# gabrieletiboni/random-envs

Hardware: NVIDIA B200
Metric: DR env-steps/sec (RandomCartPole-v0 single-step kernel, uniform DR resample on reset) (higher is better)
Workload: dtype f32

## Files before the change

### include/renv.h

```cpp
#ifndef RENV_B200_H
#define RENV_B200_H

#include <stdint.h>

#ifdef __cplusplus
extern "C" {
#endif

#define RENV_ABI_VERSION 6
#define RENV_MAX_DIM 32
#define RENV_NUM_STATS 6
#define RENV_TILE_ENVS_F32 1024
#define RENV_TILE_ENVS_F64 512
#define RENV_NUM_COUNTERS 3

enum renv_status {
    RENV_OK = 0,
    RENV_E_NULL = -1,
    RENV_E_ALIGN = -2,
    RENV_E_SIZE = -3,
    RENV_E_DIM = -4,
    RENV_E_DRTYPE = -5,
    RENV_E_INTEGRATOR = -6,
    RENV_E_ARG = -7
};

enum renv_dr_type {
    RENV_DR_NONE = 0,
    RENV_DR_UNIFORM = 1,
    RENV_DR_TRUNCNORM = 2,
    RENV_DR_GAUSSIAN = 3,
    RENV_DR_FULLGAUSSIAN = 4
};

enum renv_integrator { RENV_EULER = 0, RENV_SEMI_IMPLICIT = 1 };

typedef struct renv_dr_cfg {
    int32_t dr_type;
    int32_t dim;
    double a[RENV_MAX_DIM];
    double b[RENV_MAX_DIM];
    double lb[RENV_MAX_DIM];
    double factor[RENV_MAX_DIM * RENV_MAX_DIM];
} renv_dr_cfg;

typedef struct renv_cartpole_env {
    void *state;
    void *xi;
    int32_t *elapsed;
    uint32_t *episode;
    int32_t *beyond;
    uint16_t *elapsed16;
    uint32_t *progress;
    int64_t n;
    int64_t ld;
    uint64_t env_id0;
    uint64_t seed;
} renv_cartpole_env;

typedef struct renv_episode_log {
    void *xi;
    void *final_state;
    int32_t *length;
    uint8_t *truncated;
    int64_t *end_tick;
    int32_t *count;
    int64_t capacity;
} renv_episode_log;

int renv_abi_version(void);
const char *renv_strerror(int code);

int renv_dr_sample_f32(float *out, int64_t n, const renv_dr_cfg *cfg, uint64_t seed, uint64_t sample_id0,
                       uint32_t call, unsigned long long *violations, void *stream);
int renv_dr_sample_f64(double *out, int64_t n, const renv_dr_cfg *cfg, uint64_t seed, uint64_t sample_id0,
                       uint32_t call, unsigned long long *violations, void *stream);

int renv_cartpole_reset_f32(const renv_cartpole_env *env, const uint8_t *mask, uint64_t tick, const renv_dr_cfg *dr,
                            unsigned long long *violations, void *stream);
int renv_cartpole_reset_f64(const renv_cartpole_env *env, const uint8_t *mask, uint64_t tick, const renv_dr_cfg *dr,
                            unsigned long long *violations, void *stream);

int renv_cartpole_step_f32(const renv_cartpole_env *env, const uint8_t *action, float *reward, uint8_t *done,
                           uint8_t *truncated, int integrator, int max_steps, int auto_reset, uint64_t tick,
                           const renv_dr_cfg *dr, unsigned long long *counters, void *stream);
int renv_cartpole_step_f64(const renv_cartpole_env *env, const uint8_t *action, double *reward, uint8_t *done,
                           uint8_t *truncated, int integrator, int max_steps, int auto_reset, uint64_t tick,
                           const renv_dr_cfg *dr, unsigned long long *counters, void *stream);

int renv_cartpole_step_lean_f32(const renv_cartpole_env *env, const uint8_t *action, uint8_t *done, uint8_t *truncated,
                                int integrator, int max_steps, uint64_t tick, const renv_dr_cfg *dr,
                                unsigned long long *counters, void *stream);

typedef struct renv_obs_noise {
    void *obs;
    double std;
} renv_obs_noise;

int renv_cartpole_reset_noisy_f32(const renv_cartpole_env *env, const renv_obs_noise *noise, const uint8_t *mask,
                                  uint64_t tick, const renv_dr_cfg *dr, unsigned long long *violations, void *stream);
int renv_cartpole_reset_noisy_f64(const renv_cartpole_env *env, const renv_obs_noise *noise, const uint8_t *mask,
                                  uint64_t tick, const renv_dr_cfg *dr, unsigned long long *violations, void *stream);
int renv_cartpole_step_noisy_f32(const renv_cartpole_env *env, const renv_obs_noise *noise, const uint8_t *action,
                                 float *reward, uint8_t *done, uint8_t *truncated, int integrator, int max_steps,
                                 int auto_reset, uint64_t tick, const renv_dr_cfg *dr, unsigned long long *counters,
                                 void *stream);
int renv_cartpole_step_noisy_f64(const renv_cartpole_env *env, const renv_obs_noise *noise, const uint8_t *action,
                                 double *reward, uint8_t *done, uint8_t *truncated, int integrator, int max_steps,
                                 int auto_reset, uint64_t tick, const renv_dr_cfg *dr, unsigned long long *counters,
                                 void *stream);

int renv_cartpole_rollout_f32(const renv_cartpole_env *env, const double w[4], double b, int K, int integrator,
                              int max_steps, uint64_t tick, const renv_dr_cfg *dr, double *stats,
                              unsigned long long *violations, void *stream);
int renv_cartpole_rollout_f64(const renv_cartpole_env *env, const double w[4], double b, int K, int integrator,
                              int max_steps, uint64_t tick, const renv_dr_cfg *dr, double *stats,
                              unsigned long long *violations, void *stream);

int renv_cartpole_rollout_noisy_f32(const renv_cartpole_env *env, const renv_obs_noise *noise, const double w[4], double b,
                                    int K, int integrator, int max_steps, uint64_t tick, const renv_dr_cfg *dr,
                                    double *stats, unsigned long long *violations, void *stream);
int renv_cartpole_rollout_noisy_f64(const renv_cartpole_env *env, const renv_obs_noise *noise, const double w[4], double b,
                                    int K, int integrator, int max_steps, uint64_t tick, const renv_dr_cfg *dr,
                                    double *stats, unsigned long long *violations, void *stream);

int renv_cartpole_step_logged_f32(const renv_cartpole_env *env, const renv_episode_log *log, const uint8_t *action,
                                  float *reward, uint8_t *done, uint8_t *truncated, int integrator, int max_steps,
                                  uint64_t tick, const renv_dr_cfg *dr, unsigned long long *counters, void *stream);
int renv_cartpole_step_logged_f64(const renv_cartpole_env *env, const renv_episode_log *log, const uint8_t *action,
                                  double *reward, uint8_t *done, uint8_t *truncated, int integrator, int max_steps,
                                  uint64_t tick, const renv_dr_cfg *dr, unsigned long long *counters, void *stream);
int renv_cartpole_rollout_logged_f32(const renv_cartpole_env *env, const renv_episode_log *log, const double w[4], double b,
                                     int K, int integrator, int max_steps, uint64_t tick, const renv_dr_cfg *dr,
                                     double *stats, unsigned long long *violations, void *stream);
int renv_cartpole_rollout_logged_f64(const renv_cartpole_env *env, const renv_episode_log *log, const double w[4], double b,
                                     int K, int integrator, int max_steps, uint64_t tick, const renv_dr_cfg *dr,
                                     double *stats, unsigned long long *violations, void *stream);

#define RENV_MLP_HIDDEN 64
#define RENV_MLP_PARAM_FLOATS 4612
#define RENV_MLP_TANH 0
#define RENV_MLP_RELU 1
typedef struct renv_mlp_policy {
    const void *params;
    int32_t activation;
} renv_mlp_policy;

int renv_cartpole_policy_actions_mlp_f32(const renv_cartpole_env *env, const renv_mlp_policy *p, uint8_t *action,
                                         float *logits, void *stream);
int renv_cartpole_rollout_mlp_f32(const renv_cartpole_env *env, const renv_mlp_policy *p, int K, int integrator,
                                  int max_steps, uint64_t tick, const renv_dr_cfg *dr, double *stats,
                                  unsigned long long *violations, void *stream);
int renv_cartpole_rollout_mlp_logged_f32(const renv_cartpole_env *env, const renv_episode_log *log,
                                         const renv_mlp_policy *p, int K, int integrator, int max_steps, uint64_t tick,
                                         const renv_dr_cfg *dr, double *stats, unsigned long long *violations,
                                         void *stream);

int renv_cartpole_policy_logp_mlp_f32(const renv_cartpole_env *env, const renv_mlp_policy *p, int sample, uint64_t tick,
                                      uint8_t *action, float *logp, float *logits, void *stream);

typedef struct renv_trajectory {
    float *obs;
    uint8_t *action;
    uint8_t *done;
    float *logp;
    uint8_t *truncated;
    float *final_obs;
    int32_t capacity;
} renv_trajectory;

int renv_cartpole_collect_mlp_f32(const renv_cartpole_env *env, const renv_mlp_policy *p, const renv_trajectory *traj,
                                  int sample, int K, int integrator, int max_steps, uint64_t tick, const renv_dr_cfg *dr,
                                  double *stats, unsigned long long *violations, void *stream);
int renv_cartpole_collect_mlp_logged_f32(const renv_cartpole_env *env, const renv_episode_log *log,
                                         const renv_mlp_policy *p, const renv_trajectory *traj, int sample, int K,
                                         int integrator, int max_steps, uint64_t tick, const renv_dr_cfg *dr,
                                         double *stats, unsigned long long *violations, void *stream);

#define RENV_SCALAR_SAVE_BYTES 512
typedef struct renv_scalar_ctrl {
    uint32_t request;
    uint32_t pad0[15];
    double arg[16];
    uint64_t arg_u64[8];
    double state[4];
    double obs[4];
    double xi[4];
    double reward;
    int32_t done;
    int32_t beyond;
    uint32_t violations;
    uint32_t pad1;
    uint32_t ack;
    uint32_t exited;
    uint32_t pad2[16];
    struct renv_scalar_outcome {
        double state[4];
        double obs[4];
        double reward;
        int32_t done;
        int32_t beyond;
        uint32_t pad[12];
    } next[2];
    uint32_t next_seq;
    uint32_t pad3[15];
} renv_scalar_ctrl;
int renv_cartpole_scalar_serve(renv_scalar_ctrl *ctrl, void *save, uint32_t lease_id, uint64_t lease_ns, void *stream);

int renv_random_actions_u8(uint8_t *action, int64_t n, uint64_t env_id0, uint64_t seed, uint32_t step,
                           void *stream);

int renv_pack_flags_u8(const uint8_t *flags, uint32_t *bits, int64_t n, void *stream);

#ifdef __cplusplus
}
#endif
#endif
```

### random_envs_b200/_lib.py

```python
import ctypes
import os

_HERE = os.path.dirname(os.path.abspath(__file__))
LIB_PATH = os.environ.get("RENV_B200_LIB", os.path.join(_HERE, "librenv_b200.so"))

ABI_VERSION = 6
MAX_DIM = 32
NUM_STATS = 6
SCALAR_SAVE_BYTES = 512
COUNTER_GAUSSIAN, COUNTER_BAD_ACTION, COUNTER_ORDER_TIMEOUT = 0, 1, 2
TILE_ENVS = {'float32': 1024, 'float64': 512}
NUM_COUNTERS = 3

OK = 0
DR_NONE, DR_UNIFORM, DR_TRUNCNORM, DR_GAUSSIAN, DR_FULLGAUSSIAN = 0, 1, 2, 3, 4
DR_TYPE_IDS = {"uniform": DR_UNIFORM, "truncnorm": DR_TRUNCNORM, "gaussian": DR_GAUSSIAN,
               "fullgaussian": DR_FULLGAUSSIAN}
EULER, SEMI_IMPLICIT = 0, 1


class DrCfg(ctypes.Structure):
    _fields_ = [("dr_type", ctypes.c_int32), ("dim", ctypes.c_int32),
                ("a", ctypes.c_double * MAX_DIM), ("b", ctypes.c_double * MAX_DIM),
                ("lb", ctypes.c_double * MAX_DIM), ("factor", ctypes.c_double * (MAX_DIM * MAX_DIM))]


class CartpoleEnv(ctypes.Structure):
    _fields_ = [("state", ctypes.c_void_p), ("xi", ctypes.c_void_p), ("elapsed", ctypes.c_void_p),
                ("episode", ctypes.c_void_p), ("beyond", ctypes.c_void_p), ("elapsed16", ctypes.c_void_p),
                ("progress", ctypes.c_void_p),
                ("n", ctypes.c_int64), ("ld", ctypes.c_int64),
                ("env_id0", ctypes.c_uint64), ("seed", ctypes.c_uint64)]


class ObsNoise(ctypes.Structure):
    _fields_ = [("obs", ctypes.c_void_p), ("std", ctypes.c_double)]


class EpisodeLog(ctypes.Structure):
    _fields_ = [("xi", ctypes.c_void_p), ("final_state", ctypes.c_void_p), ("length", ctypes.c_void_p),
                ("truncated", ctypes.c_void_p), ("end_tick", ctypes.c_void_p), ("count", ctypes.c_void_p),
                ("capacity", ctypes.c_int64)]


class MlpPolicy(ctypes.Structure):
    _fields_ = [("params", ctypes.c_void_p), ("activation", ctypes.c_int32)]


class Trajectory(ctypes.Structure):
    _fields_ = [("obs", ctypes.c_void_p), ("action", ctypes.c_void_p), ("done", ctypes.c_void_p),
                ("logp", ctypes.c_void_p), ("truncated", ctypes.c_void_p), ("final_obs", ctypes.c_void_p),
                ("capacity", ctypes.c_int32)]


_vp, _i64, _u64, _u32, _int, _dbl = (ctypes.c_void_p, ctypes.c_int64, ctypes.c_uint64, ctypes.c_uint32,
                                     ctypes.c_int, ctypes.c_double)
_cfg_p, _env_p, _noise_p = ctypes.POINTER(DrCfg), ctypes.POINTER(CartpoleEnv), ctypes.POINTER(ObsNoise)
_log_p = ctypes.POINTER(EpisodeLog)
_mlp_p = ctypes.POINTER(MlpPolicy)
_traj_p = ctypes.POINTER(Trajectory)

SIGNATURES = {
    "renv_abi_version": (_int, []),
    "renv_strerror": (ctypes.c_char_p, [_int]),
    "renv_dr_sample_f32": (_int, [_vp, _i64, _cfg_p, _u64, _u64, _u32, _vp, _vp]),
    "renv_dr_sample_f64": (_int, [_vp, _i64, _cfg_p, _u64, _u64, _u32, _vp, _vp]),
    "renv_cartpole_reset_f32": (_int, [_env_p, _vp, _u64, _cfg_p, _vp, _vp]),
    "renv_cartpole_reset_f64": (_int, [_env_p, _vp, _u64, _cfg_p, _vp, _vp]),
    "renv_cartpole_step_f32": (_int, [_env_p, _vp, _vp, _vp, _vp, _int, _int, _int, _u64, _cfg_p, _vp, _vp]),
    "renv_cartpole_step_f64": (_int, [_env_p, _vp, _vp, _vp, _vp, _int, _int, _int, _u64, _cfg_p, _vp, _vp]),
    "renv_cartpole_step_lean_f32": (_int, [_env_p, _vp, _vp, _vp, _int, _int, _u64, _cfg_p, _vp, _vp]),
    "renv_cartpole_reset_noisy_f32": (_int, [_env_p, _noise_p, _vp, _u64, _cfg_p, _vp, _vp]),
    "renv_cartpole_reset_noisy_f64": (_int, [_env_p, _noise_p, _vp, _u64, _cfg_p, _vp, _vp]),
    "renv_cartpole_step_noisy_f32": (_int, [_env_p, _noise_p, _vp, _vp, _vp, _vp, _int, _int, _int, _u64, _cfg_p, _vp, _vp]),
    "renv_cartpole_step_noisy_f64": (_int, [_env_p, _noise_p, _vp, _vp, _vp, _vp, _int, _int, _int, _u64, _cfg_p, _vp, _vp]),
    "renv_cartpole_rollout_f32": (_int, [_env_p, ctypes.POINTER(_dbl), _dbl, _int, _int, _int, _u64, _cfg_p, _vp, _vp, _vp]),
    "renv_cartpole_rollout_f64": (_int, [_env_p, ctypes.POINTER(_dbl), _dbl, _int, _int, _int, _u64, _cfg_p, _vp, _vp, _vp]),
    "renv_cartpole_rollout_noisy_f32": (_int, [_env_p, _noise_p, ctypes.POINTER(_dbl), _dbl, _int, _int, _int, _u64, _cfg_p, _vp, _vp, _vp]),
    "renv_cartpole_rollout_noisy_f64": (_int, [_env_p, _noise_p, ctypes.POINTER(_dbl), _dbl, _int, _int, _int, _u64, _cfg_p, _vp, _vp, _vp]),
    "renv_cartpole_step_logged_f32": (_int, [_env_p, _log_p, _vp, _vp, _vp, _vp, _int, _int, _u64, _cfg_p, _vp, _vp]),
    "renv_cartpole_step_logged_f64": (_int, [_env_p, _log_p, _vp, _vp, _vp, _vp, _int, _int, _u64, _cfg_p, _vp, _vp]),
    "renv_cartpole_rollout_logged_f32": (_int, [_env_p, _log_p, ctypes.POINTER(_dbl), _dbl, _int, _int, _int, _u64, _cfg_p, _vp, _vp, _vp]),
    "renv_cartpole_rollout_logged_f64": (_int, [_env_p, _log_p, ctypes.POINTER(_dbl), _dbl, _int, _int, _int, _u64, _cfg_p, _vp, _vp, _vp]),
    "renv_cartpole_policy_actions_mlp_f32": (_int, [_env_p, _mlp_p, _vp, _vp, _vp]),
    "renv_cartpole_rollout_mlp_f32": (_int, [_env_p, _mlp_p, _int, _int, _int, _u64, _cfg_p, _vp, _vp, _vp]),
    "renv_cartpole_rollout_mlp_logged_f32": (_int, [_env_p, _log_p, _mlp_p, _int, _int, _int, _u64, _cfg_p, _vp, _vp, _vp]),
    "renv_cartpole_policy_logp_mlp_f32": (_int, [_env_p, _mlp_p, _int, _u64, _vp, _vp, _vp, _vp]),
    "renv_cartpole_collect_mlp_f32": (_int, [_env_p, _mlp_p, _traj_p, _int, _int, _int, _int, _u64, _cfg_p, _vp, _vp, _vp]),
    "renv_cartpole_collect_mlp_logged_f32": (_int, [_env_p, _log_p, _mlp_p, _traj_p, _int, _int, _int, _int, _u64, _cfg_p,
                                                    _vp, _vp, _vp]),
    "renv_cartpole_scalar_serve": (_int, [_vp, _vp, _u32, _u64, _vp]),
    "renv_random_actions_u8": (_int, [_vp, _i64, _u64, _u64, _u32, _vp]),
    "renv_pack_flags_u8": (_int, [_vp, _vp, _i64, _vp]),
}


class RenvError(RuntimeError):

    def __init__(self, fn, code, message):
        super().__init__("%s failed with %d: %s" % (fn, code, message))
        self.code = code


_lib = None


def load():
    global _lib
    if _lib is not None:
        return _lib
    if not os.path.isfile(LIB_PATH):
        raise ImportError(
            "random_envs_b200: %s is missing. Build it with `python -m random_envs_b200.build` "
            "(needs nvcc; sm_100a). There is no CPU fallback." % LIB_PATH)
    lib = ctypes.CDLL(LIB_PATH)
    for name, (restype, argtypes) in SIGNATURES.items():
        try:
            fn = getattr(lib, name)
        except AttributeError as exc:
            raise ImportError("random_envs_b200: symbol %s missing from %s" % (name, LIB_PATH)) from exc
        fn.restype, fn.argtypes = restype, argtypes
    if lib.renv_abi_version() != ABI_VERSION:
        raise ImportError("random_envs_b200: ABI version mismatch (library %d, binding %d); rebuild"
                          % (lib.renv_abi_version(), ABI_VERSION))
    _lib = lib
    return lib


def strerror(code):
    return load().renv_strerror(code).decode()


def call(name, *args):
    rc = getattr(load(), name)(*args)
    if rc != OK:
        raise RenvError(name, rc, strerror(rc))


def make_dr_cfg(dr_type, a, b, lb=None, factor=None):
    cfg = DrCfg()
    if dr_type is None:
        cfg.dr_type, cfg.dim = DR_NONE, 0
        return cfg
    if dr_type not in DR_TYPE_IDS:
        raise Exception("Unknown dr_type:" + str(dr_type))
    dim = len(a)
    if not 1 <= dim <= MAX_DIM:
        raise ValueError("task_dim %d outside [1, %d]" % (dim, MAX_DIM))
    cfg.dr_type, cfg.dim = DR_TYPE_IDS[dr_type], dim
    for i in range(dim):
        cfg.a[i] = float(a[i])
        cfg.b[i] = float(b[i])
        cfg.lb[i] = float(lb[i]) if lb is not None else 0.0
    if factor is not None:
        for i in range(dim):
            for k in range(dim):
                cfg.factor[i * dim + k] = float(factor[i][k])
    return cfg
```

### random_envs_b200/csrc/renv_abi.cu

```cuda
#include "../../include/renv.h"
#include "renv_kernels.cuh"
#include <cmath>
#include "renv_rollout_pair.cuh"
#include "renv_fullgauss_tc.cuh"
#include "renv_mlp_policy.cuh"
#include "renv_scalar_server.cuh"
#include <stdlib.h>

#ifndef RENV_ROLLOUT_F32_PAIR
#define RENV_ROLLOUT_F32_PAIR 1
#endif

using namespace renv;

namespace {

inline bool aligned(const void *p, size_t a) { return (reinterpret_cast<uintptr_t>(p) & (a - 1)) == 0; }

template <typename T> int to_cfg4(const renv_dr_cfg *dr, DrCfg4<T> *out)
{
    out->dr_type = kDrNone;
    out->dim = 4;
    for (int k = 0; k < 4; ++k) { out->a[k] = T(0); out->b[k] = T(0); out->floor[k] = T(0); }
    for (int k = 0; k < 16; ++k) out->factor[k] = T(0);
    if (dr == nullptr || dr->dr_type == RENV_DR_NONE) return RENV_OK;
    if (dr->dr_type < RENV_DR_NONE || dr->dr_type > RENV_DR_FULLGAUSSIAN) return RENV_E_DRTYPE;
    if (dr->dim != 4) return RENV_E_DIM;
    out->dr_type = dr->dr_type;
    for (int k = 0; k < 4; ++k) {
        const T a = (T)dr->a[k], b = (T)dr->b[k];
        out->a[k] = a;
        if (dr->dr_type == RENV_DR_UNIFORM) {
            const T width = b - a;
            out->b[k] = sizeof(T) == 4 ? (T)(width * (T)(1.0 / 16777216.0)) : width;
            out->floor[k] = T(0);
        } else if (dr->dr_type == RENV_DR_FULLGAUSSIAN) {
            out->b[k] = b;
            out->floor[k] = (T)dr->lb[k];
        } else {
            out->b[k] = b;
            out->floor[k] = dr->dr_type == RENV_DR_TRUNCNORM ? (T)dr->lb[k] : (T)0.1;
        }
    }
    if (dr->dr_type == RENV_DR_FULLGAUSSIAN)
        for (int k = 0; k < 16; ++k) out->factor[k] = (T)dr->factor[k];
    return RENV_OK;
}

enum ElapsedKind { kNeedElapsed32, kNeedElapsed16, kNeedEitherElapsed };
template <typename T>
int check_env(const renv_cartpole_env *env, bool need_beyond, EnvPtrs<T> *out, ElapsedKind elapsed = kNeedElapsed32)
{
    if (env == nullptr || env->state == nullptr || env->xi == nullptr) return RENV_E_NULL;
    if (elapsed == kNeedElapsed32 && env->elapsed == nullptr) return RENV_E_NULL;
    if (elapsed == kNeedElapsed16 && env->elapsed16 == nullptr) return RENV_E_NULL;
    if (elapsed == kNeedEitherElapsed && env->elapsed == nullptr && env->elapsed16 == nullptr) return RENV_E_NULL;
    if (need_beyond && env->beyond == nullptr) return RENV_E_NULL;
    if (env->n <= 0 || env->ld < env->n) return RENV_E_SIZE;
    constexpr int V = VecTraits<T>::V;
    if (env->ld % V != 0) return RENV_E_ALIGN;
    if (!aligned(env->state, 16) || !aligned(env->xi, 16) || !aligned(env->elapsed, 16) || !aligned(env->elapsed16, 16) ||
        (env->episode && !aligned(env->episode, 4)) || !aligned(env->progress, 8) || (env->beyond && !aligned(env->beyond, 4)))
        return RENV_E_ALIGN;
    out->state = static_cast<T *>(env->state);
    out->xi = static_cast<T *>(env->xi);
    out->elapsed = env->elapsed;
    out->elapsed16 = env->elapsed16;
    out->progress = env->progress;
    out->episode = env->episode;
    out->beyond = env->beyond;
    out->n = env->n;
    out->ld = env->ld;
    out->env_id0 = env->env_id0;
    out->seed = env->seed;
    out->obs = nullptr;
    out->noise_std = T(0);
    return RENV_OK;
}

template <typename T> int attach_noise(const renv_obs_noise *noise, EnvPtrs<T> *env)
{
    if (noise == nullptr) return RENV_OK;
    if (noise->obs == nullptr) return RENV_E_NULL;
    if (!aligned(noise->obs, 16)) return RENV_E_ALIGN;
    if (!(noise->std >= 0.0)) return RENV_E_ARG;
    env->obs = static_cast<T *>(noise->obs);
    env->noise_std = (T)noise->std;
    return RENV_OK;
}

template <typename T> int check_log(const renv_episode_log *log, LogPtrs<T> *out)
{
    if (log == nullptr || log->xi == nullptr || log->final_state == nullptr || log->length == nullptr ||
        log->truncated == nullptr || log->end_tick == nullptr || log->count == nullptr)
        return RENV_E_NULL;
    if (log->capacity < 1 || log->capacity > 0x7fffffffLL) return RENV_E_SIZE;
    if (!aligned(log->xi, 16) || !aligned(log->final_state, 16) || !aligned(log->length, 4) || !aligned(log->end_tick, 8) ||
        !aligned(log->count, 4))
        return RENV_E_ALIGN;
    out->xi = static_cast<T *>(log->xi);
    out->final_state = static_cast<T *>(log->final_state);
    out->length = log->length;
    out->truncated = log->truncated;
    out->end_tick = log->end_tick;
    out->count = log->count;
    out->capacity = (uint32_t)log->capacity;
    return RENV_OK;
}

inline int launch_status() { return (int)cudaGetLastError(); }

#ifndef RENV_STEP_PDL
#define RENV_STEP_PDL 1
#endif
template <typename Args>
int launch_pdl(void (*kernel)(const Args), unsigned blocks, unsigned threads, cudaStream_t stream, const Args &args)
{
    cudaLaunchConfig_t cfg = {};
    cfg.gridDim = dim3(blocks, 1, 1);
    cfg.blockDim = dim3(threads, 1, 1);
    cfg.dynamicSmemBytes = 0;
    cfg.stream = stream;
    cudaLaunchAttribute attr[1];
    attr[0].id = cudaLaunchAttributeProgrammaticStreamSerialization;
    attr[0].val.programmaticStreamSerializationAllowed = 1;
    cfg.attrs = attr;
    cfg.numAttrs = RENV_STEP_PDL ? 1 : 0;
    const cudaError_t rc = cudaLaunchKernelEx(&cfg, kernel, args);
    return rc != cudaSuccess ? (int)rc : launch_status();
}

template <int kType, int kStore>
void launch_sampler(float *out, int64_t n, const DrCfgPrepared<float> &c, uint64_t seed, uint64_t sample_id0, uint32_t call,
                    unsigned long long *violations, int items, unsigned blocks, cudaStream_t st)
{
    const PhiloxKeys ks = philox_keys((uint32_t)seed, (uint32_t)(seed >> 32));
    dr_sample_f32_kernel<kType, kStore><<<blocks, kSampleThreads, 0, st>>>(out, n, c, seed, ks, sample_id0, call, violations, items);
}
template <int kType, int kStore>
void launch_sampler(double *out, int64_t n, const DrCfgPrepared<double> &c, uint64_t seed, uint64_t sample_id0, uint32_t call,
                    unsigned long long *violations, int items, unsigned blocks, cudaStream_t st)
{
    if (kType == kDrUniform) {
        bool plain = true;
        for (int k = 0; k < c.dim; ++k) plain = plain && (c.b[k] == 0.0 || (std::fabs(c.b[k]) > 1e-250 && std::isfinite(c.b[k])));
        if (plain) {
            const PhiloxKeys ks = philox_keys((uint32_t)seed, (uint32_t)(seed >> 32));
            dr_sample_f64_uniform_kernel<kStore><<<blocks, kSampleThreads, 0, st>>>(out, n, c, ks, sample_id0, call, items);
            return;
        }
    }
    dr_sample_kernel<double, kType, kStore><<<blocks, kSampleThreads, 0, st>>>(out, n, c, seed, sample_id0, call, violations, items);
}

bool launch_fullgaussian_tc(double *, int64_t, const FullGaussCfg<double> &, uint64_t, uint64_t, uint32_t,
                            unsigned long long *, cudaStream_t, int *) { return false; }
bool launch_fullgaussian_tc(float *out, int64_t n, const FullGaussCfg<float> &g, uint64_t seed, uint64_t sample_id0,
                            uint32_t call, unsigned long long *counters, cudaStream_t st, int *rc)
{
    const char *knob = getenv("RENV_FULLGAUSS_TENSOR");
    if (knob && knob[0] == '0') return false;
    int dev = 0, sms = 0;
    cudaError_t e = cudaGetDevice(&dev);
    if (e == cudaSuccess) e = cudaDeviceGetAttribute(&sms, cudaDevAttrMultiProcessorCount, dev);
    if (e != cudaSuccess) { *rc = (int)e; return true; }
    const int64_t tiles = (n + kFgTile - 1) / kFgTile;
    const int64_t grid = tiles < (int64_t)sms * RENV_FG_TC_CTAS ? tiles : (int64_t)sms * RENV_FG_TC_CTAS;
    FullGaussCfg<float> gt = g;
    for (int k = 0; k < 32; ++k) {
        gt.hi[k] = g.hi[k] - g.lo[k];
        gt.mean[k] = 0.25f * g.mean[k];
    }
    const PhiloxKeys ks = philox_keys((uint32_t)seed, (uint32_t)(seed >> 32));
    dr_sample_fullgaussian_tc_kernel<<<(unsigned)grid, kFgThreads, kFgPadSmem, st>>>(out, n, gt, ks, sample_id0, call, counters);
    *rc = launch_status();
    return true;
}

template <typename T>
int dr_sample(T *out, int64_t n, const renv_dr_cfg *cfg, uint64_t seed, uint64_t sample_id0, uint32_t call,
              unsigned long long *violations, void *stream)
{
    int rc_tc = RENV_OK;
    if (out == nullptr || cfg == nullptr) return RENV_E_NULL;
    if (n <= 0) return RENV_E_SIZE;
    if (cfg->dim < 1 || cfg->dim > RENV_MAX_DIM) return RENV_E_DIM;
    if (cfg->dr_type < RENV_DR_UNIFORM || cfg->dr_type > RENV_DR_FULLGAUSSIAN) return RENV_E_DRTYPE;
    if (!aligned(out, 16)) return RENV_E_ALIGN;
    if (cfg->dr_type == RENV_DR_FULLGAUSSIAN) {
        FullGaussCfg<T> g;
        g.dim = cfg->dim;
        for (int k = 0; k < 32; ++k) {
            const bool ok = k < cfg->dim;
            g.mean[k] = ok ? (T)cfg->a[k] : T(0); g.lo[k] = ok ? (T)cfg->b[k] : T(0); g.hi[k] = ok ? (T)cfg->lb[k] : T(0);
        }
        for (int k = 0; k < 32; ++k)
            for (int d = 0; d < 32; ++d)
                g.ft[k * 32 + d] = (k < cfg->dim && d < cfg->dim) ? (T)cfg->factor[d * cfg->dim + k] : T(0);
        const int64_t gblocks = (n + kFullGaussThreads - 1) / kFullGaussThreads;
        if (gblocks > 0x7fffffffLL) return RENV_E_SIZE;
        const cudaStream_t gst = static_cast<cudaStream_t>(stream);
        if (cfg->dim > 16 && launch_fullgaussian_tc(out, n, g, seed, sample_id0, call, violations, gst, &rc_tc)) return rc_tc;
        if (cfg->dim <= 4) dr_sample_fullgaussian_kernel<T, 4><<<(unsigned)gblocks, kFullGaussThreads, 0, gst>>>(out, n, g, seed, sample_id0, call);
        else if (cfg->dim <= 8) dr_sample_fullgaussian_kernel<T, 8><<<(unsigned)gblocks, kFullGaussThreads, 0, gst>>>(out, n, g, seed, sample_id0, call);
        else if (cfg->dim <= 16) dr_sample_fullgaussian_kernel<T, 16><<<(unsigned)gblocks, kFullGaussThreads, 0, gst>>>(out, n, g, seed, sample_id0, call);
        else dr_sample_fullgaussian_kernel<T, 32><<<(unsigned)gblocks, kFullGaussThreads, 0, gst>>>(out, n, g, seed, sample_id0, call);
        return launch_status();
    }
    DrCfgPrepared<T> c;
    c.dr_type = cfg->dr_type;
    c.dim = cfg->dim;
    for (int k = 0; k < 32; ++k) {
        const bool ok = k < cfg->dim;
        const T a = ok ? (T)cfg->a[k] : T(0), b = ok ? (T)cfg->b[k] : T(0);
        c.a[k] = a;
        if (cfg->dr_type == RENV_DR_UNIFORM) {
            const T width = b - a;
            c.b[k] = sizeof(T) == 4 ? (T)(width * (T)(1.0 / 16777216.0)) : (T)width;
        } else {
            c.b[k] = b;
        }
        c.floor[k] = !ok ? T(0) : cfg->dr_type == RENV_DR_TRUNCNORM ? (T)cfg->lb[k] : (T)0.1;
    }
    const int items = sampler_items<T>(n, cfg->dim);
    const int kTile = tile_samples<T>(cfg->dim, items);
    const int64_t blocks = (n + kTile - 1) / kTile;
    if (blocks > 0x7fffffffLL) return RENV_E_SIZE;
    constexpr int P = Pack<T>::kPerBlock;
    const int store = cfg->dim % P == 0 ? 0 : (sizeof(T) == 4 && cfg->dim % 2 == 0 ? 1 : 2);
    const cudaStream_t st = static_cast<cudaStream_t>(stream);
#define RENV_LAUNCH_SAMPLER(TYPE, STORE) launch_sampler<TYPE, STORE>(out, n, c, seed, sample_id0, call, violations, items, (unsigned)blocks, st)
#define RENV_LAUNCH_SAMPLER_TYPE(TYPE) \
    do { if (store == 0) RENV_LAUNCH_SAMPLER(TYPE, 0); else if (store == 1) RENV_LAUNCH_SAMPLER(TYPE, 1); \
         else RENV_LAUNCH_SAMPLER(TYPE, 2); } while (0)
    if (cfg->dr_type == RENV_DR_UNIFORM) RENV_LAUNCH_SAMPLER_TYPE(kDrUniform);
    else if (cfg->dr_type == RENV_DR_TRUNCNORM) RENV_LAUNCH_SAMPLER_TYPE(kDrTruncnorm);
    else RENV_LAUNCH_SAMPLER_TYPE(kDrGaussian);
#undef RENV_LAUNCH_SAMPLER_TYPE
#undef RENV_LAUNCH_SAMPLER
    return launch_status();
}

template <typename T>
int cartpole_reset(const renv_cartpole_env *env, const renv_obs_noise *noise, const uint8_t *mask, uint64_t tick,
                   const renv_dr_cfg *dr, unsigned long long *violations, void *stream)
{
    ResetArgs<T> a;
    int rc = check_env<T>(env, false, &a.env, kNeedEitherElapsed);
    if (rc) return rc;
    rc = attach_noise<T>(noise, &a.env);
    if (rc) return rc;
    rc = to_cfg4<T>(dr, &a.dr);
    if (rc) return rc;
    a.mask = mask;
    a.tick = tick;
    a.violations = violations;
    const int64_t blocks = (env->n + 255) / 256;
    if (blocks > 0x7fffffffLL) return RENV_E_SIZE;
    cartpole_reset_kernel<T><<<(unsigned)blocks, 256, 0, static_cast<cudaStream_t>(stream)>>>(a);
    return launch_status();
}

template <typename T, bool kLean>
int cartpole_step(const renv_cartpole_env *env, const renv_obs_noise *noise, const uint8_t *action, T *reward,
                  uint8_t *done, uint8_t *truncated, int integrator, int max_steps, int auto_reset, uint64_t tick,
                  const renv_dr_cfg *dr, unsigned long long *counters, void *stream,
                  const renv_episode_log *log = nullptr, bool logged = false)
{
    StepArgs<T> a;
    int rc = check_env<T>(env, !auto_reset, &a.env, kLean ? kNeedElapsed16 : kNeedElapsed32);
    if (rc) return rc;
    rc = attach_noise<T>(noise, &a.env);
    if (rc) return rc;
    LoggedStepArgs<T> la;
    if (logged && (rc = check_log<T>(log, &la.log))) return rc;
    if (action == nullptr || done == nullptr) return RENV_E_NULL;
    if (reward == nullptr && !auto_reset) return RENV_E_NULL;
    if (!aligned(action, 4) || !aligned(reward, 16) || !aligned(done, 4) || (truncated && !aligned(truncated, 4)))
        return RENV_E_ALIGN;
    if (counters && !aligned(counters, 8)) return RENV_E_ALIGN;
    if (integrator != RENV_EULER && integrator != RENV_SEMI_IMPLICIT) return RENV_E_INTEGRATOR;
    if (kLean && max_steps > 65535) return RENV_E_SIZE;
    rc = to_cfg4<T>(auto_reset ? dr : nullptr, &a.dr);
    if (rc) return rc;
    a.action = action; a.reward = reward; a.done = done; a.truncated = truncated;
    a.euler = integrator == RENV_EULER;
    a.max_steps = max_steps;
    a.tick = tick;
    a.counters = counters;
    constexpr int64_t per_block = (int64_t)kStepThreads * VecTraits<T>::V;
    const int64_t blocks = (env->n + per_block - 1) / per_block;
    if (blocks > 0x7fffffffLL) return RENV_E_SIZE;
    const cudaStream_t st = static_cast<cudaStream_t>(stream);
    const bool noisy = a.env.obs != nullptr;
    if (logged) {
        la.step = a;
        return launch_pdl(cartpole_step_logged_kernel<T>, (unsigned)blocks, kStepThreads, st, la);
    }
    if (kLean) return launch_pdl(cartpole_step_kernel<T, true, false, true>, (unsigned)blocks, kStepThreads, st, a);
    if (auto_reset && !noisy) return launch_pdl(cartpole_step_kernel<T, true, false>, (unsigned)blocks, kStepThreads, st, a);
    if (auto_reset) return launch_pdl(cartpole_step_kernel<T, true, true>, (unsigned)blocks, kStepThreads, st, a);
    if (!noisy) return launch_pdl(cartpole_step_kernel<T, false, false>, (unsigned)blocks, kStepThreads, st, a);
    return launch_pdl(cartpole_step_kernel<T, false, true>, (unsigned)blocks, kStepThreads, st, a);
}

template <typename T> int launch_rollout_random(const RolloutArgs<T> &a, cudaStream_t stream)
{
    const int64_t blocks = (a.env.n + kRolloutThreads - 1) / kRolloutThreads;
    if (blocks > 0x7fffffffLL) return RENV_E_SIZE;
    if (a.euler) cartpole_rollout_kernel<T, true, false, true><<<(unsigned)blocks, kRolloutThreads, 0, stream>>>(a);
    else cartpole_rollout_kernel<T, false, false, true><<<(unsigned)blocks, kRolloutThreads, 0, stream>>>(a);
    return launch_status();
}
template <typename T> int launch_rollout_random(const LoggedRolloutArgs<T> &a, cudaStream_t stream)
{
    const int64_t blocks = (a.roll.env.n + kRolloutThreads - 1) / kRolloutThreads;
    if (blocks > 0x7fffffffLL) return RENV_E_SIZE;
    if (a.roll.euler) cartpole_rollout_logged_kernel<T, true, true><<<(unsigned)blocks, kRolloutThreads, 0, stream>>>(a);
    else cartpole_rollout_logged_kernel<T, false, true><<<(unsigned)blocks, kRolloutThreads, 0, stream>>>(a);
    return launch_status();
}
template <typename T> int launch_rollout_noisy(const RolloutArgs<T> &a, cudaStream_t stream)
{
    const int64_t blocks = (a.env.n + kRolloutThreads - 1) / kRolloutThreads;
    if (blocks > 0x7fffffffLL) return RENV_E_SIZE;
    if (a.euler) cartpole_rollout_kernel<T, true, true><<<(unsigned)blocks, kRolloutThreads, 0, stream>>>(a);
    else cartpole_rollout_kernel<T, false, true><<<(unsigned)blocks, kRolloutThreads, 0, stream>>>(a);
    return launch_status();
}
int launch_rollout(const RolloutArgs<double> &a, cudaStream_t stream)
{
    if (a.env.obs) return launch_rollout_noisy(a, stream);
    const int64_t blocks = (a.env.n + kRolloutThreads - 1) / kRolloutThreads;
    if (blocks > 0x7fffffffLL) return RENV_E_SIZE;
    if (a.euler) cartpole_rollout_kernel<double, true><<<(unsigned)blocks, kRolloutThreads, 0, stream>>>(a);
    else cartpole_rollout_kernel<double, false><<<(unsigned)blocks, kRolloutThreads, 0, stream>>>(a);
    return launch_status();
}
int launch_rollout(const RolloutArgs<float> &a, cudaStream_t stream)
{
    if (a.env.obs) return launch_rollout_noisy(a, stream);
#if RENV_ROLLOUT_F32_PAIR
    const int64_t threads = (a.env.n + kPairSlots - 1) / kPairSlots;
    const int64_t blocks = (threads + kRolloutThreads - 1) / kRolloutThreads;
    if (blocks > 0x7fffffffLL) return RENV_E_SIZE;
    if (a.euler) cartpole_rollout_pair_kernel<true><<<(unsigned)blocks, kRolloutThreads, 0, stream>>>(a);
    else cartpole_rollout_pair_kernel<false><<<(unsigned)blocks, kRolloutThreads, 0, stream>>>(a);
#else
    const int64_t blocks = (a.env.n + kRolloutThreads - 1) / kRolloutThreads;
    if (blocks > 0x7fffffffLL) return RENV_E_SIZE;
    if (a.euler) cartpole_rollout_kernel<float, true><<<(unsigned)blocks, kRolloutThreads, 0, stream>>>(a);
    else cartpole_rollout_kernel<float, false><<<(unsigned)blocks, kRolloutThreads, 0, stream>>>(a);
#endif
    return launch_status();
}
int launch_rollout(const LoggedRolloutArgs<double> &a, cudaStream_t stream)
{
    const int64_t blocks = (a.roll.env.n + kRolloutThreads - 1) / kRolloutThreads;
    if (blocks > 0x7fffffffLL) return RENV_E_SIZE;
    if (a.roll.euler) cartpole_rollout_logged_kernel<double, true, false><<<(unsigned)blocks, kRolloutThreads, 0, stream>>>(a);
    else cartpole_rollout_logged_kernel<double, false, false><<<(unsigned)blocks, kRolloutThreads, 0, stream>>>(a);
    return launch_status();
}
int launch_rollout(const LoggedRolloutArgs<float> &a, cudaStream_t stream)
{
    const int64_t threads = (a.roll.env.n + kPairSlots - 1) / kPairSlots;
    const int64_t blocks = (threads + kRolloutThreads - 1) / kRolloutThreads;
    if (blocks > 0x7fffffffLL) return RENV_E_SIZE;
    if (a.roll.euler) cartpole_rollout_pair_logged_kernel<true><<<(unsigned)blocks, kRolloutThreads, 0, stream>>>(a);
    else cartpole_rollout_pair_logged_kernel<false><<<(unsigned)blocks, kRolloutThreads, 0, stream>>>(a);
    return launch_status();
}

template <typename T>
int cartpole_rollout(const renv_cartpole_env *env, const renv_obs_noise *noise, const double w[4], double b, int K,
                     int integrator, int max_steps, uint64_t tick, const renv_dr_cfg *dr, double *stats,
                     unsigned long long *violations, void *stream, const renv_episode_log *log = nullptr,
                     bool logged = false)
{
    RolloutArgs<T> a;
    int rc = check_env<T>(env, false, &a.env);
    if (rc) return rc;
    rc = attach_noise<T>(noise, &a.env);
    if (rc) return rc;
    LoggedRolloutArgs<T> la;
    if (logged && (rc = check_log<T>(log, &la.log))) return rc;
    if (stats == nullptr) return RENV_E_NULL;
    if (w == nullptr && noise != nullptr) return RENV_E_ARG;
    if (!aligned(stats, 8)) return RENV_E_ALIGN;
    if (K <= 0 || K > (1 << 30)) return RENV_E_SIZE;
    if (integrator != RENV_EULER && integrator != RENV_SEMI_IMPLICIT) return RENV_E_INTEGRATOR;
    rc = to_cfg4<T>(dr, &a.dr);
    if (rc) return rc;
    a.policy = w ? Policy<T>{ (T)w[0], (T)w[1], (T)w[2], (T)w[3], (T)b } : Policy<T>{ T(0), T(0), T(0), T(0), T(0) };
    a.K = K;
    a.euler = integrator == RENV_EULER;
    a.max_steps = max_steps;
    a.tick = tick;
    a.stats = stats;
    a.violations = violations;
    const cudaStream_t st = static_cast<cudaStream_t>(stream);
    if (logged) {
        la.roll = a;
        return w == nullptr ? launch_rollout_random(la, st) : launch_rollout(la, st);
    }
    if (w == nullptr) return launch_rollout_random(a, st);
    return launch_rollout(a, st);
}

int check_mlp(const renv_mlp_policy *p)
{
    if (p == nullptr || p->params == nullptr) return RENV_E_NULL;
    if (!aligned(p->params, 16)) return RENV_E_ALIGN;
    if (p->activation != RENV_MLP_TANH && p->activation != RENV_MLP_RELU) return RENV_E_ARG;
    return RENV_OK;
}

int sm_count(int *sms)
{
    int dev = 0;
    cudaError_t e = cudaGetDevice(&dev);
    if (e == cudaSuccess) e = cudaDeviceGetAttribute(sms, cudaDevAttrMultiProcessorCount, dev);
    return (int)e;
}

int policy_actions_mlp(const renv_cartpole_env *env, const renv_mlp_policy *p, uint8_t *action, float *logits, void *stream)
{
    if (env == nullptr || env->state == nullptr) return RENV_E_NULL;
    int rc = check_mlp(p);
    if (rc) return rc;
    if (action == nullptr) return RENV_E_NULL;
    if (env->n <= 0 || env->ld < env->n) return RENV_E_SIZE;
    if (env->ld % 4 != 0 || !aligned(env->state, 16) || !aligned(action, 4) || !aligned(logits, 16)) return RENV_E_ALIGN;
    MlpActionArgs a;
    a.state = static_cast<const float *>(env->state);
    a.n = env->n; a.ld = env->ld;
    a.params = static_cast<const float *>(p->params);
    a.action = action; a.logits = logits;
    int sms = 0;
    if ((rc = sm_count(&sms))) return rc;
    const int64_t tiles = (env->n + kMlpThreads - 1) / kMlpThreads;
    const int64_t grid = tiles < (int64_t)sms * RENV_MLP_CTAS ? tiles : (int64_t)sms * RENV_MLP_CTAS;
    const cudaStream_t st = static_cast<cudaStream_t>(stream);
    if (p->activation == RENV_MLP_TANH) cartpole_policy_actions_mlp_kernel<kMlpTanh><<<(unsigned)grid, kMlpThreads, 0, st>>>(a);
    else cartpole_policy_actions_mlp_kernel<kMlpRelu><<<(unsigned)grid, kMlpThreads, 0, st>>>(a);
    return launch_status();
}

template <int kAct, bool kLog> void launch_rollout_mlp(const MlpRolloutArgs &a, unsigned blocks, cudaStream_t st)
{
    if (a.roll.euler) cartpole_rollout_mlp_kernel<kAct, true, kLog><<<blocks, kMlpThreads, 0, st>>>(a);
    else cartpole_rollout_mlp_kernel<kAct, false, kLog><<<blocks, kMlpThreads, 0, st>>>(a);
}

int prepare_rollout_mlp(const renv_cartpole_env *env, const renv_episode_log *log, bool logged, const renv_mlp_policy *p,
                        int K, int integrator, int max_steps, uint64_t tick, const renv_dr_cfg *dr, double *stats,
                        unsigned long long *violations, MlpRolloutArgs *a)
{
    int rc = check_env<float>(env, false, &a->roll.env);
    if (rc) return rc;
    if (logged && (rc = check_log<float>(log, &a->log))) return rc;
    if (!logged) a->log = LogPtrs<float>{};
    if ((rc = check_mlp(p))) return rc;
    if (stats == nullptr) return RENV_E_NULL;
    if (!aligned(stats, 8)) return RENV_E_ALIGN;
    if (K <= 0 || K > (1 << 30)) return RENV_E_SIZE;
    if (integrator != RENV_EULER && integrator != RENV_SEMI_IMPLICIT) return RENV_E_INTEGRATOR;
    if ((rc = to_cfg4<float>(dr, &a->roll.dr))) return rc;
    a->roll.policy = Policy<float>{ 0.0f, 0.0f, 0.0f, 0.0f, 0.0f };
    a->roll.K = K;
    a->roll.euler = integrator == RENV_EULER;
    a->roll.max_steps = max_steps;
    a->roll.tick = tick;
    a->roll.stats = stats;
    a->roll.violations = violations;
    a->params = static_cast<const float *>(p->params);
    const int64_t blocks = (env->n + kMlpThreads - 1) / kMlpThreads;
    if (blocks > 0x7fffffffLL) return RENV_E_SIZE;
    return RENV_OK;
}

int rollout_mlp(const renv_cartpole_env *env, const renv_episode_log *log, bool logged, const renv_mlp_policy *p, int K,
                int integrator, int max_steps, uint64_t tick, const renv_dr_cfg *dr, double *stats,
                unsigned long long *violations, void *stream)
{
    MlpRolloutArgs a;
    const int rc = prepare_rollout_mlp(env, log, logged, p, K, integrator, max_steps, tick, dr, stats, violations, &a);
    if (rc) return rc;
    const unsigned blocks = (unsigned)((env->n + kMlpThreads - 1) / kMlpThreads);
    const cudaStream_t st = static_cast<cudaStream_t>(stream);
    if (p->activation == RENV_MLP_TANH) {
        if (logged) launch_rollout_mlp<kMlpTanh, true>(a, blocks, st);
        else launch_rollout_mlp<kMlpTanh, false>(a, blocks, st);
    } else {
        if (logged) launch_rollout_mlp<kMlpRelu, true>(a, blocks, st);
        else launch_rollout_mlp<kMlpRelu, false>(a, blocks, st);
    }
    return launch_status();
}

int policy_logp_mlp(const renv_cartpole_env *env, const renv_mlp_policy *p, int sample, uint64_t tick, uint8_t *action,
                    float *logp, float *logits, void *stream)
{
    if (env == nullptr || env->state == nullptr) return RENV_E_NULL;
    int rc = check_mlp(p);
    if (rc) return rc;
    if (action == nullptr) return RENV_E_NULL;
    if (env->n <= 0 || env->ld < env->n) return RENV_E_SIZE;
    if (env->ld % 4 != 0 || !aligned(env->state, 16) || !aligned(action, 4) || !aligned(logits, 16) || !aligned(logp, 4))
        return RENV_E_ALIGN;
    if (sample != 0 && sample != 1) return RENV_E_ARG;
    MlpLogpArgs a;
    a.act.state = static_cast<const float *>(env->state);
    a.act.n = env->n; a.act.ld = env->ld;
    a.act.params = static_cast<const float *>(p->params);
    a.act.action = action; a.act.logits = logits;
    a.logp = logp;
    a.env_id0 = env->env_id0; a.seed = env->seed; a.tick = tick;
    a.sample = sample;
    int sms = 0;
    if ((rc = sm_count(&sms))) return rc;
    const int64_t tiles = (env->n + kMlpThreads - 1) / kMlpThreads;
    const int64_t grid = tiles < (int64_t)sms * RENV_MLP_ROLLOUT_CTAS ? tiles : (int64_t)sms * RENV_MLP_ROLLOUT_CTAS;
    const cudaStream_t st = static_cast<cudaStream_t>(stream);
    if (p->activation == RENV_MLP_TANH) cartpole_policy_logp_mlp_kernel<kMlpTanh><<<(unsigned)grid, kMlpThreads, 0, st>>>(a);
    else cartpole_policy_logp_mlp_kernel<kMlpRelu><<<(unsigned)grid, kMlpThreads, 0, st>>>(a);
    return launch_status();
}

int check_traj(const renv_trajectory *t, int K, MlpTrajPtrs *out)
{
    if (t == nullptr || t->obs == nullptr || t->action == nullptr || t->done == nullptr) return RENV_E_NULL;
    if (!aligned(t->obs, 16) || !aligned(t->final_obs, 16) || !aligned(t->action, 4) || !aligned(t->done, 4) ||
        !aligned(t->logp, 4) || !aligned(t->truncated, 4))
        return RENV_E_ALIGN;
    if (K > t->capacity) return RENV_E_ARG;
    *out = MlpTrajPtrs{ t->obs, t->action, t->done, t->logp, t->truncated, t->final_obs };
    return RENV_OK;
}

template <int kAct, bool kLog> void launch_collect_mlp(const MlpCollectArgs &a, unsigned blocks, cudaStream_t st)
{
    if (a.roll.euler) cartpole_collect_mlp_kernel<kAct, true, kLog><<<blocks, kMlpThreads, 0, st>>>(a);
    else cartpole_collect_mlp_kernel<kAct, false, kLog><<<blocks, kMlpThreads, 0, st>>>(a);
}

int collect_mlp(const renv_cartpole_env *env, const renv_episode_log *log, bool logged, const renv_mlp_policy *p,
                const renv_trajectory *traj, int sample, int K, int integrator, int max_steps, uint64_t tick,
                const renv_dr_cfg *dr, double *stats, unsigned long long *violations, void *stream)
{
    MlpRolloutArgs r;
    int rc = prepare_rollout_mlp(env, log, logged, p, K, integrator, max_steps, tick, dr, stats, violations, &r);
    if (rc) return rc;
    MlpCollectArgs a;
    if ((rc = check_traj(traj, K, &a.traj))) return rc;
    if (sample != 0 && sample != 1) return RENV_E_ARG;
    a.roll = r.roll; a.params = r.params; a.log = r.log;
    a.sample = sample;
    const unsigned blocks = (unsigned)((env->n + kMlpThreads - 1) / kMlpThreads);
    const cudaStream_t st = static_cast<cudaStream_t>(stream);
    if (p->activation == RENV_MLP_TANH) {
        if (logged) launch_collect_mlp<kMlpTanh, true>(a, blocks, st);
        else launch_collect_mlp<kMlpTanh, false>(a, blocks, st);
    } else {
        if (logged) launch_collect_mlp<kMlpRelu, true>(a, blocks, st);
        else launch_collect_mlp<kMlpRelu, false>(a, blocks, st);
    }
    return launch_status();
}

}

extern "C" {

int renv_abi_version(void) { return RENV_ABI_VERSION; }

const char *renv_strerror(int code)
{
    switch (code) {
    case RENV_OK: return "ok";
    case RENV_E_NULL: return "required pointer is NULL";
    case RENV_E_ALIGN: return "pointer or ld violates the alignment contract (16 B data, 4 B byte arrays, ld % V)";
    case RENV_E_SIZE: return "invalid size (n <= 0, ld < n, K <= 0 or grid too large)";
    case RENV_E_DIM: return "dim outside [1, 32] (cart-pole needs 4)";
    case RENV_E_DRTYPE: return "Unknown dr_type";
    case RENV_E_INTEGRATOR: return "unknown integrator";
    case RENV_E_ARG: return "invalid argument";
    default: return code > 0 ? cudaGetErrorString((cudaError_t)code) : "unknown renv status";
    }
}

int renv_dr_sample_f32(float *out, int64_t n, const renv_dr_cfg *cfg, uint64_t seed, uint64_t sample_id0, uint32_t call,
                       unsigned long long *violations, void *stream)
{
    return dr_sample<float>(out, n, cfg, seed, sample_id0, call, violations, stream);
}
int renv_dr_sample_f64(double *out, int64_t n, const renv_dr_cfg *cfg, uint64_t seed, uint64_t sample_id0,
                       uint32_t call, unsigned long long *violations, void *stream)
{
    return dr_sample<double>(out, n, cfg, seed, sample_id0, call, violations, stream);
}

int renv_cartpole_reset_f32(const renv_cartpole_env *env, const uint8_t *mask, uint64_t tick, const renv_dr_cfg *dr,
                            unsigned long long *violations, void *stream)
{
    return cartpole_reset<float>(env, nullptr, mask, tick, dr, violations, stream);
}
int renv_cartpole_reset_f64(const renv_cartpole_env *env, const uint8_t *mask, uint64_t tick, const renv_dr_cfg *dr,
                            unsigned long long *violations, void *stream)
{
    return cartpole_reset<double>(env, nullptr, mask, tick, dr, violations, stream);
}

int renv_cartpole_step_f32(const renv_cartpole_env *env, const uint8_t *action, float *reward, uint8_t *done,
                           uint8_t *truncated, int integrator, int max_steps, int auto_reset, uint64_t tick,
                           const renv_dr_cfg *dr, unsigned long long *counters, void *stream)
{
    return cartpole_step<float, false>(env, nullptr, action, reward, done, truncated, integrator, max_steps, auto_reset,
                                       tick, dr, counters, stream);
}
int renv_cartpole_step_lean_f32(const renv_cartpole_env *env, const uint8_t *action, uint8_t *done, uint8_t *truncated,
                                int integrator, int max_steps, uint64_t tick, const renv_dr_cfg *dr,
                                unsigned long long *counters, void *stream)
{
    return cartpole_step<float, true>(env, nullptr, action, nullptr, done, truncated, integrator, max_steps, 1, tick, dr,
                                      counters, stream);
}
int renv_cartpole_step_f64(const renv_cartpole_env *env, const uint8_t *action, double *reward, uint8_t *done,
                           uint8_t *truncated, int integrator, int max_steps, int auto_reset, uint64_t tick,
                           const renv_dr_cfg *dr, unsigned long long *violations, void *stream)
{
    return cartpole_step<double, false>(env, nullptr, action, reward, done, truncated, integrator, max_steps, auto_reset, tick,
                                 dr, violations, stream);
}

int renv_cartpole_reset_noisy_f32(const renv_cartpole_env *env, const renv_obs_noise *noise, const uint8_t *mask,
                                  uint64_t tick, const renv_dr_cfg *dr, unsigned long long *violations, void *stream)
{
    if (noise == nullptr) return RENV_E_NULL;
    return cartpole_reset<float>(env, noise, mask, tick, dr, violations, stream);
}
int renv_cartpole_reset_noisy_f64(const renv_cartpole_env *env, const renv_obs_noise *noise, const uint8_t *mask,
                                  uint64_t tick, const renv_dr_cfg *dr, unsigned long long *violations, void *stream)
{
    if (noise == nullptr) return RENV_E_NULL;
    return cartpole_reset<double>(env, noise, mask, tick, dr, violations, stream);
}
int renv_cartpole_step_noisy_f32(const renv_cartpole_env *env, const renv_obs_noise *noise, const uint8_t *action,
                                 float *reward, uint8_t *done, uint8_t *truncated, int integrator, int max_steps,
                                 int auto_reset, uint64_t tick, const renv_dr_cfg *dr, unsigned long long *violations,
                                 void *stream)
{
    if (noise == nullptr) return RENV_E_NULL;
    return cartpole_step<float, false>(env, noise, action, reward, done, truncated, integrator, max_steps, auto_reset, tick,
                                dr, violations, stream);
}
int renv_cartpole_step_noisy_f64(const renv_cartpole_env *env, const renv_obs_noise *noise, const uint8_t *action,
                                 double *reward, uint8_t *done, uint8_t *truncated, int integrator, int max_steps,
                                 int auto_reset, uint64_t tick, const renv_dr_cfg *dr, unsigned long long *violations,
                                 void *stream)
{
    if (noise == nullptr) return RENV_E_NULL;
    return cartpole_step<double, false>(env, noise, action, reward, done, truncated, integrator, max_steps, auto_reset, tick,
                                 dr, violations, stream);
}

int renv_cartpole_rollout_f32(const renv_cartpole_env *env, const double w[4], double b, int K, int integrator,
                              int max_steps, uint64_t tick, const renv_dr_cfg *dr, double *stats,
                              unsigned long long *violations, void *stream)
{
    return cartpole_rollout<float>(env, nullptr, w, b, K, integrator, max_steps, tick, dr, stats, violations, stream);
}
int renv_cartpole_rollout_f64(const renv_cartpole_env *env, const double w[4], double b, int K, int integrator,
                              int max_steps, uint64_t tick, const renv_dr_cfg *dr, double *stats,
                              unsigned long long *violations, void *stream)
{
    return cartpole_rollout<double>(env, nullptr, w, b, K, integrator, max_steps, tick, dr, stats, violations, stream);
}

int renv_cartpole_step_logged_f32(const renv_cartpole_env *env, const renv_episode_log *log, const uint8_t *action,
                                  float *reward, uint8_t *done, uint8_t *truncated, int integrator, int max_steps,
                                  uint64_t tick, const renv_dr_cfg *dr, unsigned long long *counters, void *stream)
{
    return cartpole_step<float, false>(env, nullptr, action, reward, done, truncated, integrator, max_steps, 1, tick, dr,
                                       counters, stream, log, true);
}
int renv_cartpole_step_logged_f64(const renv_cartpole_env *env, const renv_episode_log *log, const uint8_t *action,
                                  double *reward, uint8_t *done, uint8_t *truncated, int integrator, int max_steps,
                                  uint64_t tick, const renv_dr_cfg *dr, unsigned long long *counters, void *stream)
{
    return cartpole_step<double, false>(env, nullptr, action, reward, done, truncated, integrator, max_steps, 1, tick, dr,
                                        counters, stream, log, true);
}
int renv_cartpole_rollout_logged_f32(const renv_cartpole_env *env, const renv_episode_log *log, const double w[4], double b,
                                     int K, int integrator, int max_steps, uint64_t tick, const renv_dr_cfg *dr,
                                     double *stats, unsigned long long *violations, void *stream)
{
    return cartpole_rollout<float>(env, nullptr, w, b, K, integrator, max_steps, tick, dr, stats, violations, stream, log,
                                   true);
}
int renv_cartpole_rollout_logged_f64(const renv_cartpole_env *env, const renv_episode_log *log, const double w[4], double b,
                                     int K, int integrator, int max_steps, uint64_t tick, const renv_dr_cfg *dr,
                                     double *stats, unsigned long long *violations, void *stream)
{
    return cartpole_rollout<double>(env, nullptr, w, b, K, integrator, max_steps, tick, dr, stats, violations, stream, log,
                                    true);
}

int renv_cartpole_rollout_noisy_f32(const renv_cartpole_env *env, const renv_obs_noise *noise, const double w[4], double b,
                                    int K, int integrator, int max_steps, uint64_t tick, const renv_dr_cfg *dr,
                                    double *stats, unsigned long long *violations, void *stream)
{
    if (noise == nullptr) return RENV_E_NULL;
    return cartpole_rollout<float>(env, noise, w, b, K, integrator, max_steps, tick, dr, stats, violations, stream);
}
int renv_cartpole_rollout_noisy_f64(const renv_cartpole_env *env, const renv_obs_noise *noise, const double w[4], double b,
                                    int K, int integrator, int max_steps, uint64_t tick, const renv_dr_cfg *dr,
                                    double *stats, unsigned long long *violations, void *stream)
{
    if (noise == nullptr) return RENV_E_NULL;
    return cartpole_rollout<double>(env, noise, w, b, K, integrator, max_steps, tick, dr, stats, violations, stream);
}

int renv_cartpole_policy_actions_mlp_f32(const renv_cartpole_env *env, const renv_mlp_policy *p, uint8_t *action,
                                         float *logits, void *stream)
{
    return policy_actions_mlp(env, p, action, logits, stream);
}
int renv_cartpole_rollout_mlp_f32(const renv_cartpole_env *env, const renv_mlp_policy *p, int K, int integrator,
                                  int max_steps, uint64_t tick, const renv_dr_cfg *dr, double *stats,
                                  unsigned long long *violations, void *stream)
{
    return rollout_mlp(env, nullptr, false, p, K, integrator, max_steps, tick, dr, stats, violations, stream);
}
int renv_cartpole_rollout_mlp_logged_f32(const renv_cartpole_env *env, const renv_episode_log *log,
                                         const renv_mlp_policy *p, int K, int integrator, int max_steps, uint64_t tick,
                                         const renv_dr_cfg *dr, double *stats, unsigned long long *violations,
                                         void *stream)
{
    return rollout_mlp(env, log, true, p, K, integrator, max_steps, tick, dr, stats, violations, stream);
}
int renv_cartpole_policy_logp_mlp_f32(const renv_cartpole_env *env, const renv_mlp_policy *p, int sample, uint64_t tick,
                                      uint8_t *action, float *logp, float *logits, void *stream)
{
    return policy_logp_mlp(env, p, sample, tick, action, logp, logits, stream);
}
int renv_cartpole_collect_mlp_f32(const renv_cartpole_env *env, const renv_mlp_policy *p, const renv_trajectory *traj,
                                  int sample, int K, int integrator, int max_steps, uint64_t tick, const renv_dr_cfg *dr,
                                  double *stats, unsigned long long *violations, void *stream)
{
    return collect_mlp(env, nullptr, false, p, traj, sample, K, integrator, max_steps, tick, dr, stats, violations, stream);
}
int renv_cartpole_collect_mlp_logged_f32(const renv_cartpole_env *env, const renv_episode_log *log,
                                         const renv_mlp_policy *p, const renv_trajectory *traj, int sample, int K,
                                         int integrator, int max_steps, uint64_t tick, const renv_dr_cfg *dr,
                                         double *stats, unsigned long long *violations, void *stream)
{
    return collect_mlp(env, log, true, p, traj, sample, K, integrator, max_steps, tick, dr, stats, violations, stream);
}

int renv_cartpole_scalar_serve(renv_scalar_ctrl *ctrl, void *save, uint32_t lease_id, uint64_t lease_ns, void *stream)
{
    if (ctrl == nullptr || save == nullptr) return RENV_E_NULL;
    if (!aligned(ctrl, 64) || !aligned(save, 16)) return RENV_E_ALIGN;
    if (lease_ns == 0 || lease_ns > 1000000000ull) return RENV_E_ARG;
    cartpole_scalar_server_kernel<<<1, 32, 0, static_cast<cudaStream_t>(stream)>>>(ctrl, static_cast<ScalarSave *>(save),
                                                                                 lease_id, lease_ns);
    return launch_status();
}

int renv_random_actions_u8(uint8_t *action, int64_t n, uint64_t env_id0, uint64_t seed, uint32_t step, void *stream)
{
    if (action == nullptr) return RENV_E_NULL;
    if (n <= 0) return RENV_E_SIZE;
    if (!aligned(action, 4)) return RENV_E_ALIGN;
    const int64_t threads = (n + 3) / 4;
    const int64_t blocks = (threads + 255) / 256;
    if (blocks > 0x7fffffffLL) return RENV_E_SIZE;
    random_actions_kernel<<<(unsigned)blocks, 256, 0, static_cast<cudaStream_t>(stream)>>>(action, n, env_id0, seed, step);
    return launch_status();
}

int renv_pack_flags_u8(const uint8_t *flags, uint32_t *bits, int64_t n, void *stream)
{
    if (flags == nullptr || bits == nullptr) return RENV_E_NULL;
    if (n <= 0) return RENV_E_SIZE;
    if (!aligned(flags, 4) || !aligned(bits, 4)) return RENV_E_ALIGN;
    const int64_t threads = (n + 31) / 32;
    const int64_t blocks = (threads + 255) / 256;
    if (blocks > 0x7fffffffLL) return RENV_E_SIZE;
    pack_flags_kernel<<<(unsigned)blocks, 256, 0, static_cast<cudaStream_t>(stream)>>>(flags, bits, n);
    return launch_status();
}

}
```

### random_envs_b200/csrc/renv_cartpole.cuh

```cuda
#pragma once
#include "renv_dr.cuh"

namespace renv {

constexpr double kForceMag = 10.0;
constexpr double kPolemassLength = 0.05;
constexpr double kTau = 0.02;
constexpr double kXThreshold = 2.4;
constexpr double kThetaThreshold = 0.20943951023931953;
constexpr double kFourThirds = 4.0 / 3.0;

template <typename T> struct Xi { T gravity, cart_mass, pole_mass, pole_length; };
template <typename T> struct State { T x, x_dot, theta, theta_dot; };

template <typename T> struct Derived;
template <> struct Derived<double> {
    double total_mass;
    double inv_total;
};
template <> struct Derived<float> {
    float force_over_total;
    float pml_over_total;
    float len_four_thirds;
    float len_pm_over_total;
};

__device__ __forceinline__ float rcp_approx(float x)
{
    float r;
    asm("rcp.approx.ftz.f32 %0, %1;" : "=f"(r) : "f"(x));
    return r;
}

constexpr float kSmallAngle = 0.25f;
template <bool kKnownSmall = false>
__device__ __forceinline__ void sincos_small(float x, float *sn, float *cs)
{
    if (kKnownSmall || fabsf(x) <= kSmallAngle) {
        const float x2 = __fmul_rn(x, x);
        const float ps = fmaf(x2, 1.0f / 120.0f, -1.0f / 6.0f);
        *sn = fmaf(__fmul_rn(x, x2), ps, x);
        float pc = fmaf(x2, -1.0f / 720.0f, 1.0f / 24.0f);
        pc = fmaf(x2, pc, -0.5f);
        *cs = fmaf(x2, pc, 1.0f);
    } else {
        sincosf(x, sn, cs);
    }
}

constexpr double kSmallAngleF64 = 0.25;
static __constant__ double kF64[20] = {
    1.0 / 6227020800.0, -1.0 / 39916800.0, 1.0 / 362880.0, -1.0 / 5040.0, 1.0 / 120.0, -1.0 / 6.0,
    1.0 / 479001600.0, -1.0 / 3628800.0, 1.0 / 40320.0, -1.0 / 720.0, 1.0 / 24.0, -0.5,
    kTau, kPolemassLength, kFourThirds, kForceMag, kXThreshold, kThetaThreshold, 1.0, 0.0 };
template <bool kKnownSmall = false>
__device__ __forceinline__ void sincos_small(double x, double *sn, double *cs)
{
    if (kKnownSmall || fabs(x) <= kSmallAngleF64) {
        const double x2 = __dmul_rn(x, x);
        double p = kF64[0];
#pragma unroll
        for (int k = 1; k < 6; ++k) p = __fma_rn(p, x2, kF64[k]);
        *sn = __fma_rn(__dmul_rn(x, x2), p, x);
        double q = kF64[6];
#pragma unroll
        for (int k = 7; k < 12; ++k) q = __fma_rn(q, x2, kF64[k]);
        *cs = __fma_rn(x2, q, kF64[18]);
    } else {
        sincos(x, sn, cs);
    }
}

__device__ __forceinline__ Derived<double> derive(const Xi<double> &p)
{
    Derived<double> d;
    d.total_mass = __dadd_rn(p.pole_mass, p.cart_mass);
    d.inv_total = __drcp_rn(d.total_mass);
    return d;
}

__device__ __forceinline__ double div_total(double a, const Derived<double> &d)
{
    const double q = __dmul_rn(a, d.inv_total);
    const double r = __fma_rn(-q, d.total_mass, a);
    return __fma_rn(r, d.inv_total, q);
}
__device__ __forceinline__ Derived<float> derive(const Xi<float> &p)
{
    Derived<float> d;
    const float inv_total_mass = rcp_approx(__fadd_rn(p.pole_mass, p.cart_mass));
    d.force_over_total = __fmul_rn((float)kForceMag, inv_total_mass);
    d.pml_over_total = __fmul_rn((float)kPolemassLength, inv_total_mass);
    d.len_four_thirds = __fmul_rn(p.pole_length, (float)kFourThirds);
    d.len_pm_over_total = __fmul_rn(p.pole_length, __fmul_rn(p.pole_mass, inv_total_mass));
    return d;
}

template <bool kKnownSmall = false>
__device__ __forceinline__ bool dynamics(State<double> &s, const Xi<double> &p, const Derived<double> &d, int action,
                                         bool euler)
{
    const double force = action == 1 ? kF64[15] : -kF64[15];
    double sn, cs;
    sincos_small<kKnownSmall>(s.theta, &sn, &cs);
    const double temp = div_total(
        __dadd_rn(force, __dmul_rn(__dmul_rn(kF64[13], __dmul_rn(s.theta_dot, s.theta_dot)), sn)), d);
    const double num = __dsub_rn(__dmul_rn(p.gravity, sn), __dmul_rn(cs, temp));
    const double den = __dmul_rn(
        p.pole_length, __dsub_rn(kF64[14], div_total(__dmul_rn(p.pole_mass, __dmul_rn(cs, cs)), d)));
    const double theta_acc = __ddiv_rn(num, den);
    const double x_acc = __dsub_rn(temp, div_total(__dmul_rn(__dmul_rn(kF64[13], theta_acc), cs), d));
    const double tau = kF64[12];
    if (euler) {
        s.x = __dadd_rn(s.x, __dmul_rn(tau, s.x_dot));
        s.x_dot = __dadd_rn(s.x_dot, __dmul_rn(tau, x_acc));
        s.theta = __dadd_rn(s.theta, __dmul_rn(tau, s.theta_dot));
        s.theta_dot = __dadd_rn(s.theta_dot, __dmul_rn(tau, theta_acc));
    } else {
        s.x_dot = __dadd_rn(s.x_dot, __dmul_rn(tau, x_acc));
        s.x = __dadd_rn(s.x, __dmul_rn(tau, s.x_dot));
        s.theta_dot = __dadd_rn(s.theta_dot, __dmul_rn(tau, theta_acc));
        s.theta = __dadd_rn(s.theta, __dmul_rn(tau, s.theta_dot));
    }
    return s.x < -kF64[16] || s.x > kF64[16] || s.theta < -kF64[17] || s.theta > kF64[17];
}

template <bool kKnownSmall = false>
__device__ __forceinline__ bool dynamics(State<float> &s, const Xi<float> &p, const Derived<float> &d, int action,
                                         bool euler)
{
    float sn, cs;
    sincos_small<kKnownSmall>(s.theta, &sn, &cs);
    const float push = action == 1 ? d.force_over_total : -d.force_over_total;
    const float temp = fmaf(__fmul_rn(__fmul_rn(s.theta_dot, s.theta_dot), sn), d.pml_over_total, push);
    const float num = fmaf(p.gravity, sn, -__fmul_rn(cs, temp));
    const float den = fmaf(-d.len_pm_over_total, __fmul_rn(cs, cs), d.len_four_thirds);
    const float theta_acc = __fmul_rn(num, rcp_approx(den));
    const float x_acc = fmaf(-__fmul_rn(d.pml_over_total, cs), theta_acc, temp);
    const float tau = (float)kTau;
    if (euler) {
        s.x = fmaf(tau, s.x_dot, s.x);
        s.x_dot = fmaf(tau, x_acc, s.x_dot);
        s.theta = fmaf(tau, s.theta_dot, s.theta);
        s.theta_dot = fmaf(tau, theta_acc, s.theta_dot);
    } else {
        s.x_dot = fmaf(tau, x_acc, s.x_dot);
        s.x = fmaf(tau, s.x_dot, s.x);
        s.theta_dot = fmaf(tau, theta_acc, s.theta_dot);
        s.theta = fmaf(tau, s.theta_dot, s.theta);
    }
    return s.x < -(float)kXThreshold || s.x > (float)kXThreshold || s.theta < -(float)kThetaThreshold ||
           s.theta > (float)kThetaThreshold;
}

template <typename T> struct Policy { T w0, w1, w2, w3, b; };

__device__ __forceinline__ int policy_action(const Policy<double> &q, const State<double> &s)
{
    double acc = __dmul_rn(q.w0, s.x);
    acc = __dadd_rn(acc, __dmul_rn(q.w1, s.x_dot));
    acc = __dadd_rn(acc, __dmul_rn(q.w2, s.theta));
    acc = __dadd_rn(acc, __dmul_rn(q.w3, s.theta_dot));
    acc = __dadd_rn(acc, q.b);
    return acc > 0.0;
}
__device__ __forceinline__ int policy_action(const Policy<float> &q, const State<float> &s)
{
    float acc = fmaf(q.w0, s.x, q.b);
    acc = fmaf(q.w1, s.x_dot, acc);
    acc = fmaf(q.w2, s.theta, acc);
    acc = fmaf(q.w3, s.theta_dot, acc);
    return acc > 0.0f;
}

__device__ __forceinline__ void init_state(State<float> &s, uint64_t seed, uint64_t id, uint64_t tick)
{
    float u[4];
    Pack<float>::uniforms(draw_block(seed, id, tick, kInit, 0), u);
    s.x = fmaf(0.1f, u[0], -0.05f);
    s.x_dot = fmaf(0.1f, u[1], -0.05f);
    s.theta = fmaf(0.1f, u[2], -0.05f);
    s.theta_dot = fmaf(0.1f, u[3], -0.05f);
}
__device__ __forceinline__ void init_state(State<double> &s, uint64_t seed, uint64_t id, uint64_t tick)
{
    double u[2], v[2];
    Pack<double>::uniforms(draw_block(seed, id, tick, kInit, 0), u);
    Pack<double>::uniforms(draw_block(seed, id, tick, kInit, 1), v);
    s.x = __dadd_rn(-0.05, __dmul_rn(0.1, u[0]));
    s.x_dot = __dadd_rn(-0.05, __dmul_rn(0.1, u[1]));
    s.theta = __dadd_rn(-0.05, __dmul_rn(0.1, v[0]));
    s.theta_dot = __dadd_rn(-0.05, __dmul_rn(0.1, v[1]));
}

__device__ __forceinline__ void add_obs_noise(const State<float> &s, float std, uint64_t seed, uint64_t id, uint64_t tick,
                                              uint32_t which, float o[4])
{
    float z[4];
    Num<float>::normals(draw_block(seed, id, tick, kObs, which * 16u), z);
    o[0] = fmaf(std, z[0], s.x); o[1] = fmaf(std, z[1], s.x_dot);
    o[2] = fmaf(std, z[2], s.theta); o[3] = fmaf(std, z[3], s.theta_dot);
}
__device__ __forceinline__ void add_obs_noise(const State<double> &s, double std, uint64_t seed, uint64_t id, uint64_t tick,
                                              uint32_t which, double o[4])
{
    double z[4];
    Pack<double>::normals(draw_block(seed, id, tick, kObs, which * 16u), z);
    Pack<double>::normals(draw_block(seed, id, tick, kObs, which * 16u + 1u), z + 2);
    o[0] = __dadd_rn(s.x, __dmul_rn(std, z[0])); o[1] = __dadd_rn(s.x_dot, __dmul_rn(std, z[1]));
    o[2] = __dadd_rn(s.theta, __dmul_rn(std, z[2])); o[3] = __dadd_rn(s.theta_dot, __dmul_rn(std, z[3]));
}

template <typename T>
__device__ __noinline__ void fullgaussian_xi(const DrCfg4<T> *cfg, uint64_t seed, uint64_t id, uint64_t tick, T *v)
{
    constexpr int P = Pack<T>::kPerBlock;
    T z[4];
#pragma unroll
    for (int j = 0; j < 4 / P; ++j) Num<T>::normals(draw_block(seed, id, tick, kXi, (uint32_t)j), z + j * P);
#pragma unroll
    for (int d = 0; d < 4; ++d) {
        T x = cfg->a[d];
#pragma unroll
        for (int k = 0; k < 4; ++k) x = Num<T>::affine(cfg->factor[d * 4 + k], z[k], x);
        v[d] = denormalize(x, cfg->b[d], cfg->floor[d]);
    }
}

template <typename T>
__device__ __forceinline__ unsigned sample_xi(Xi<T> &p, const DrCfg4<T> &cfg, uint64_t seed, uint64_t id, uint64_t tick)
{
    constexpr int P = Pack<T>::kPerBlock;
    T v[4] = { p.gravity, p.cart_mass, p.pole_mass, p.pole_length };
    unsigned violations = 0;
    if (cfg.dr_type == kDrFullGaussian) {
        fullgaussian_xi<T>(&cfg, seed, id, tick, v);
    } else {
#pragma unroll
        for (int j = 0; j < 4 / P; ++j) violations += sample_dim_block<T>(cfg, seed, id, tick, kXi, j, v + j * P);
    }
    p.gravity = v[0]; p.cart_mass = v[1]; p.pole_mass = v[2]; p.pole_length = v[3];
    return violations;
}

}
```

### random_envs_b200/csrc/renv_kernels.cuh

```cuda
#pragma once
#include <cuda_runtime.h>
#include "renv_cartpole.cuh"

namespace renv {

template <typename T> struct VecTraits;
template <> struct VecTraits<float> {
    static constexpr int V = 4;
    using Real = float4; using Int = int4; using Byte = uchar4; using Half = ushort4;
};
template <> struct VecTraits<double> {
    static constexpr int V = 2;
    using Real = double2; using Int = int2; using Byte = uchar2; using Half = ushort2;
};

__device__ __forceinline__ bool full_tile(int64_t block0, int64_t n, int tile) { return block0 + tile <= n; }

template <typename Vec, typename S, int V> __device__ __forceinline__ void vload(S (&dst)[V], const S *src)
{
    static_assert(sizeof(Vec) == sizeof(S) * V, "vector width");
    const Vec v = *reinterpret_cast<const Vec *>(src);
    const S *e = reinterpret_cast<const S *>(&v);
#pragma unroll
    for (int k = 0; k < V; ++k) dst[k] = e[k];
}
template <typename Vec, typename S, int V> __device__ __forceinline__ void vstore(S *dst, const S (&src)[V])
{
    Vec v;
    S *e = reinterpret_cast<S *>(&v);
#pragma unroll
    for (int k = 0; k < V; ++k) e[k] = src[k];
    *reinterpret_cast<Vec *>(dst) = v;
}

__device__ __forceinline__ Xi<float> load_xi(const float *xi, int64_t i)
{
    const float4 v = *reinterpret_cast<const float4 *>(xi + 4 * i);
    return Xi<float>{ v.x, v.y, v.z, v.w };
}
__device__ __forceinline__ Xi<double> load_xi(const double *xi, int64_t i)
{
    const double2 a = *reinterpret_cast<const double2 *>(xi + 4 * i), b = *reinterpret_cast<const double2 *>(xi + 4 * i + 2);
    return Xi<double>{ a.x, a.y, b.x, b.y };
}
__device__ __forceinline__ void store_xi(float *xi, int64_t i, const Xi<float> &p)
{
    *reinterpret_cast<float4 *>(xi + 4 * i) = make_float4(p.gravity, p.cart_mass, p.pole_mass, p.pole_length);
}
__device__ __forceinline__ void store_xi(double *xi, int64_t i, const Xi<double> &p)
{
    *reinterpret_cast<double2 *>(xi + 4 * i) = make_double2(p.gravity, p.cart_mass);
    *reinterpret_cast<double2 *>(xi + 4 * i + 2) = make_double2(p.pole_mass, p.pole_length);
}

template <typename T> struct EnvPtrs {
    T *state; T *xi; int32_t *elapsed; uint32_t *episode; int32_t *beyond;
    uint16_t *elapsed16;
    uint32_t *progress;
    int64_t n, ld; uint64_t env_id0, seed;
    T *obs; T noise_std;
};

template <typename T>
__device__ __forceinline__ unsigned reset_env(const EnvPtrs<T> &env, const DrCfg4<T> &dr, int64_t i, uint64_t tick, uint64_t seed)
{
    const int64_t ld = env.ld;
    const uint64_t id = env.env_id0 + (uint64_t)i;
    State<T> st;
    init_state(st, seed, id, tick);
    env.state[0 * ld + i] = st.x; env.state[1 * ld + i] = st.x_dot;
    env.state[2 * ld + i] = st.theta; env.state[3 * ld + i] = st.theta_dot;
    if (env.obs) {
        T o[4];
        add_obs_noise(st, env.noise_std, seed, id, tick, 1u, o);
        env.obs[0 * ld + i] = o[0]; env.obs[1 * ld + i] = o[1]; env.obs[2 * ld + i] = o[2]; env.obs[3 * ld + i] = o[3];
    }
    unsigned viol = 0;
    if (dr.dr_type != kDrNone) {
        Xi<T> xi = { T(0), T(0), T(0), T(0) };
        viol = sample_xi(xi, dr, seed, id, tick);
        store_xi(env.xi, i, xi);
    }
    if (env.episode) atomicAdd(env.episode + i, 1u);
    return viol;
}

template <typename T> struct LogPtrs {
    T *xi; T *final_state; int32_t *length; uint8_t *truncated; int64_t *end_tick; int32_t *count;
    uint32_t capacity;
};

template <typename T> __device__ __forceinline__ bool beyond_thresholds(const State<T> &s)
{
    return s.x < -(T)kXThreshold || s.x > (T)kXThreshold || s.theta < -(T)kThetaThreshold || s.theta > (T)kThetaThreshold;
}

template <typename T>
__device__ __forceinline__ void log_episode(const LogPtrs<T> &log, int64_t ld, int64_t i, uint32_t count, const Xi<T> &xi,
                                            const State<T> &s, int32_t length, bool truncated, uint64_t tick)
{
    const int64_t r = (int64_t)(count % log.capacity) * ld + i;
    store_xi(log.xi, r, xi);
    store_xi(log.final_state, r, Xi<T>{ s.x, s.x_dot, s.theta, s.theta_dot });
    log.length[r] = length;
    log.truncated[r] = truncated ? 1 : 0;
    log.end_tick[r] = (int64_t)tick;
}

enum Counter : int { kCounterGaussian = 0, kCounterBadAction = 1, kCounterOrderTimeout = 2 };

__device__ __forceinline__ uint32_t ld_acquire_gpu(const uint32_t *p)
{
    uint32_t v;
    asm volatile("ld.acquire.gpu.global.u32 %0, [%1];" : "=r"(v) : "l"(p) : "memory");
    return v;
}
__device__ __forceinline__ void st_release_gpu(uint32_t *p, uint32_t v)
{
    asm volatile("st.release.gpu.global.u32 [%0], %1;" :: "l"(p), "r"(v) : "memory");
}
__device__ __forceinline__ void prefetch_l2(const void *p, uint32_t bytes)
{
    asm volatile("cp.async.bulk.prefetch.L2.global [%0], %1;" :: "l"(p), "r"(bytes) : "memory");
}
#ifndef RENV_ORDER_SPINS
#define RENV_ORDER_SPINS (1 << 21)
#endif
#ifndef RENV_TILE_PREFETCH
#define RENV_TILE_PREFETCH 1
#endif

template <typename T> struct StepArgs {
    EnvPtrs<T> env;
    const uint8_t *action; T *reward; uint8_t *done; uint8_t *truncated;
    int euler, max_steps;
    uint64_t tick;
    DrCfg4<T> dr;
    unsigned long long *counters;
};

#ifndef RENV_STEP_THREADS
#define RENV_STEP_THREADS 256
#endif
constexpr int kStepThreads = RENV_STEP_THREADS;
#ifndef RENV_STEP_MIN_CTAS
#define RENV_STEP_MIN_CTAS(T) ((sizeof(T) == 4 ? 4 : 3) * 256 / kStepThreads)
#endif

template <typename T, bool kAutoReset, bool kNoisy = false, bool kLean = false>
__global__ void __launch_bounds__(kStepThreads, kNoisy ? (sizeof(T) == 8 ? 2 : 3) : RENV_STEP_MIN_CTAS(T)) cartpole_step_kernel(const __grid_constant__ StepArgs<T> a)
{
    constexpr bool kLog = false;
    const LogPtrs<T> log = {};
#include "renv_step_body.cuh"
}

template <typename T> struct LoggedStepArgs { StepArgs<T> step; LogPtrs<T> log; };

template <typename T>
__global__ void __launch_bounds__(kStepThreads, RENV_STEP_MIN_CTAS(T)) cartpole_step_logged_kernel(const __grid_constant__ LoggedStepArgs<T> args)
{
    constexpr bool kAutoReset = true, kNoisy = false, kLean = false, kLog = true;
    const StepArgs<T> &a = args.step;
    const LogPtrs<T> &log = args.log;
#include "renv_step_body.cuh"
}

template <typename T> struct ResetArgs {
    EnvPtrs<T> env;
    const uint8_t *mask;
    uint64_t tick;
    DrCfg4<T> dr;
    unsigned long long *violations;
};

template <typename T> __global__ void __launch_bounds__(256) cartpole_reset_kernel(const __grid_constant__ ResetArgs<T> a)
{
    const int64_t i = (int64_t)blockIdx.x * blockDim.x + threadIdx.x;
    if (i >= a.env.n) return;
    if (a.mask && !a.mask[i]) return;
    if (a.env.elapsed) a.env.elapsed[i] = 0;
    if (a.env.elapsed16) a.env.elapsed16[i] = 0;
    if (a.env.beyond) a.env.beyond[i] = -1;
    const unsigned viol = reset_env(a.env, a.dr, i, a.tick, a.env.seed);
    if (viol && a.violations) atomicAdd(a.violations, (unsigned long long)viol);
}

__device__ __forceinline__ void atomic_min_f64(double *addr, double v)
{
    unsigned long long *p = reinterpret_cast<unsigned long long *>(addr);
    unsigned long long old = *p;
    while (v < __longlong_as_double((long long)old)) {
        const unsigned long long seen = atomicCAS(p, old, (unsigned long long)__double_as_longlong(v));
        if (seen == old) break;
        old = seen;
    }
}
__device__ __forceinline__ void atomic_max_f64(double *addr, double v)
{
    unsigned long long *p = reinterpret_cast<unsigned long long *>(addr);
    unsigned long long old = *p;
    while (v > __longlong_as_double((long long)old)) {
        const unsigned long long seen = atomicCAS(p, old, (unsigned long long)__double_as_longlong(v));
        if (seen == old) break;
        old = seen;
    }
}

constexpr int kRolloutThreads = 256;

__device__ __forceinline__ void rollout_publish(double *stats, unsigned long long *violations, unsigned episodes,
                                                unsigned sum_len, unsigned sum_r_u, unsigned long long sum_r2_u,
                                                float min_r, float max_r, unsigned viol)
{
    double sum_r = (double)sum_r_u, sum_r2 = (double)sum_r2_u;
    double cnt = (double)episodes, len = (double)sum_len;
#pragma unroll
    for (int off = 16; off > 0; off >>= 1) {
        cnt += __shfl_xor_sync(0xffffffffu, cnt, off);
        len += __shfl_xor_sync(0xffffffffu, len, off);
        sum_r += __shfl_xor_sync(0xffffffffu, sum_r, off);
        sum_r2 += __shfl_xor_sync(0xffffffffu, sum_r2, off);
        min_r = fminf(min_r, __shfl_xor_sync(0xffffffffu, min_r, off));
        max_r = fmaxf(max_r, __shfl_xor_sync(0xffffffffu, max_r, off));
        viol += __shfl_xor_sync(0xffffffffu, viol, off);
    }
    __shared__ double sh[kRolloutThreads / 32][4];
    __shared__ float shm[kRolloutThreads / 32][2];
    __shared__ unsigned shv[kRolloutThreads / 32];
    const int warp = threadIdx.x >> 5, lane = threadIdx.x & 31;
    if (lane == 0) {
        sh[warp][0] = cnt; sh[warp][1] = sum_r; sh[warp][2] = sum_r2; sh[warp][3] = len;
        shm[warp][0] = min_r; shm[warp][1] = max_r; shv[warp] = viol;
    }
    __syncthreads();
    if (threadIdx.x == 0) {
        const int nw = blockDim.x >> 5;
        for (int w = 1; w < nw; ++w) {
            cnt += sh[w][0]; sum_r += sh[w][1]; sum_r2 += sh[w][2]; len += sh[w][3];
            min_r = fminf(min_r, shm[w][0]); max_r = fmaxf(max_r, shm[w][1]); viol += shv[w];
        }
        if (cnt > 0.0) {
            atomicAdd(stats + 0, cnt);
            atomicAdd(stats + 1, sum_r);
            atomicAdd(stats + 2, sum_r2);
            atomic_min_f64(stats + 3, (double)min_r);
            atomic_max_f64(stats + 4, (double)max_r);
            atomicAdd(stats + 5, len);
        }
        if (viol && violations) atomicAdd(violations, (unsigned long long)viol);
    }
}

template <typename T> struct RolloutArgs {
    EnvPtrs<T> env;
    Policy<T> policy;
    int K, euler, max_steps;
    uint64_t tick;
    DrCfg4<T> dr;
    double *stats;
    unsigned long long *violations;
};

struct ActionBits { uint4 r; uint32_t group; };
template <typename T> struct RolloutThread {
    State<T> s; Xi<T> p; Derived<T> d;
    int32_t el; uint32_t new_episodes; bool xi_dirty;
    int remaining;
    int parked;
    State<T> obs0; bool obs_loaded; uint32_t after_reset;
    unsigned long long sum_r2; unsigned sum_r; float min_r, max_r; unsigned episodes, sum_len, viol;
    ActionBits act;
    bool refresh;
};

#ifndef RENV_RESET_BATCH
#define RENV_RESET_BATCH 4
#endif
#ifndef RENV_STEPS_PER_CHECK
#define RENV_STEPS_PER_CHECK 8
#endif
#ifndef RENV_UNROLL_F64
#define RENV_UNROLL_F64 2
#endif
constexpr int kResetBatch = RENV_RESET_BATCH;
constexpr int kStepsPerCheck = RENV_STEPS_PER_CHECK;
constexpr int kUnrollF64 = RENV_UNROLL_F64;
#ifndef RENV_RANDOM_RESET_BATCH
#define RENV_RANDOM_RESET_BATCH 8
#endif
#ifndef RENV_RANDOM_STEPS_PER_CHECK
#define RENV_RANDOM_STEPS_PER_CHECK 16
#endif
#ifndef RENV_RANDOM_UNROLL
#define RENV_RANDOM_UNROLL RENV_UNROLL_F64
#endif
constexpr int kRandomUnroll = RENV_RANDOM_UNROLL;
#ifndef RENV_ROLLOUT_F64_CTAS
#define RENV_ROLLOUT_F64_CTAS 3
#endif

__device__ __forceinline__ uint32_t action_bit(const uint4 &r, uint32_t step)
{
    const bool hi = (step & 64u) != 0u;
    const uint64_t half = (uint64_t)(hi ? r.w : r.y) << 32 | (uint64_t)(hi ? r.z : r.x);
    return (uint32_t)(half >> (step & 63u)) & 1u;
}
template <typename T, bool kEuler, bool kKnownSmall, bool kNoisy = false, bool kRandom = false>
__device__ __forceinline__ void rollout_step(RolloutThread<T> &t, const RolloutArgs<T> &a, const Policy<T> &policy,
                                             int32_t limit, uint64_t id = 0)
{
    int action;
    uint32_t step = 0u;
    if (kRandom) {
        step = (uint32_t)a.tick + (uint32_t)(a.K - t.remaining);
        action = (int)action_bit(t.act.r, step);
    } else if (kNoisy) {
        State<T> o = t.obs0;
        if (!t.obs_loaded) {
            T ov[4];
            const uint64_t tick_now = a.tick + (uint64_t)(a.K - t.remaining);
            add_obs_noise(t.s, a.env.noise_std, a.env.seed, id, tick_now - 1, t.after_reset, ov);
            o = State<T>{ ov[0], ov[1], ov[2], ov[3] };
        }
        t.obs_loaded = false; t.after_reset = 0u;
        action = policy_action(policy, o);
    } else {
        action = policy_action(policy, t.s);
    }
    const bool terminated = dynamics<kKnownSmall>(t.s, t.p, t.d, action, kEuler);
    t.el += 1;
    const bool ended = terminated || t.el >= limit;
    bool park = ended;
    if (kRandom) {
        const bool cross = ((step + 1u) & 127u) == 0u;
        t.refresh = cross && !ended;
        park = ended || cross;
    }
    t.parked = park ? t.remaining - 1 : t.parked;
    t.remaining = park ? 0 : t.remaining - 1;
}

template <typename T, bool kRandom = false>
__device__ __forceinline__ void rollout_reset(RolloutThread<T> &t, const RolloutArgs<T> &a, uint64_t id)
{
    if (!(kRandom && t.refresh)) {
        const float ret = (float)t.el;
        t.episodes += 1; t.sum_len += (unsigned)t.el;
        t.sum_r += (unsigned)t.el; t.sum_r2 += (unsigned long long)t.el * (unsigned)t.el;
        t.min_r = fminf(t.min_r, ret); t.max_r = fmaxf(t.max_r, ret);
        t.new_episodes += 1; t.el = 0;
        const uint64_t reset_tick = a.tick + (uint64_t)(a.K - t.parked - 1);
        if (a.dr.dr_type != kDrNone) {
            t.p = Xi<T>{ T(0), T(0), T(0), T(0) };
            t.viol += sample_xi(t.p, a.dr, a.env.seed, id, reset_tick);
            t.d = derive(t.p);
            t.xi_dirty = true;
        }
        init_state(t.s, a.env.seed, id, reset_tick);
        t.after_reset = 1u;
    }
    if (kRandom) {
        const uint32_t group = ((uint32_t)a.tick + (uint32_t)(a.K - t.parked)) >> 7;
        if (group != t.act.group) {
            t.act.group = group;
            t.act.r = draw_block(a.env.seed, id, (uint64_t)group, kAction, 0);
        }
        t.refresh = false;
    }
    t.remaining = t.parked;
    t.parked = -1;
}

__device__ __forceinline__ float pin(float v) { asm volatile("" : "+f"(v)); return v; }
__device__ __forceinline__ double pin(double v) { asm volatile("" : "+d"(v)); return v; }

#define RENV_ROLLOUT_CTAS(T, kNoisy, kRandom) (sizeof(T) == 4 ? 3 : ((kNoisy) || (kRandom)) ? 2 : RENV_ROLLOUT_F64_CTAS)

template <typename T, bool kEuler, bool kNoisy = false, bool kRandom = false>
__global__ void __launch_bounds__(kRolloutThreads, RENV_ROLLOUT_CTAS(T, kNoisy, kRandom))
cartpole_rollout_kernel(const __grid_constant__ RolloutArgs<T> a)
{
    constexpr bool kLog = false;
    const LogPtrs<T> log = {};
#include "renv_rollout_body.cuh"
}

template <typename T> struct LoggedRolloutArgs { RolloutArgs<T> roll; LogPtrs<T> log; };

template <typename T, bool kEuler, bool kRandom>
__global__ void __launch_bounds__(kRolloutThreads, RENV_ROLLOUT_CTAS(T, false, kRandom))
cartpole_rollout_logged_kernel(const __grid_constant__ LoggedRolloutArgs<T> args)
{
    constexpr bool kNoisy = false, kLog = true;
    const RolloutArgs<T> &a = args.roll;
    const LogPtrs<T> &log = args.log;
#include "renv_rollout_body.cuh"
}

__device__ __forceinline__ uint32_t nibble_of(uint32_t v)
{
    return ((__vcmpne4(v, 0u) & 0x08040201u) * 0x01010101u) >> 24;
}
__global__ void __launch_bounds__(256)
pack_flags_kernel(const uint8_t *__restrict__ flags, uint32_t *__restrict__ bits, int64_t n)
{
    const int64_t w = (int64_t)blockIdx.x * blockDim.x + threadIdx.x;
    const int64_t i0 = w * 32;
    if (i0 >= n) return;
    uint32_t out = 0u;
    if (i0 + 32 <= n && (reinterpret_cast<uintptr_t>(flags) & 15u) == 0u) {
        const uint4 a = __ldg(reinterpret_cast<const uint4 *>(flags + i0));
        const uint4 b = __ldg(reinterpret_cast<const uint4 *>(flags + i0) + 1);
        out = nibble_of(a.x) | nibble_of(a.y) << 4 | nibble_of(a.z) << 8 | nibble_of(a.w) << 12 |
              nibble_of(b.x) << 16 | nibble_of(b.y) << 20 | nibble_of(b.z) << 24 | nibble_of(b.w) << 28;
    } else {
        for (int k = 0; k < 32 && i0 + k < n; ++k) out |= (flags[i0 + k] != 0 ? 1u : 0u) << k;
    }
    bits[w] = out;
}

constexpr int kSampleThreads = 256;
constexpr int kSamplerItemsMin = 4, kSamplerItemsMax = 32;
template <typename T> __host__ __device__ inline int sampler_log2pad(int dim)
{
    const int blocks_per_sample = (dim + (int)(16 / sizeof(T)) - 1) / (int)(16 / sizeof(T));
    int log2pad = 0;
    while ((1 << log2pad) < blocks_per_sample) ++log2pad;
    return log2pad;
}
template <typename T> inline int sampler_items(int64_t n, int dim)
{
    const int64_t work = n << sampler_log2pad<T>(dim);
    const int64_t per_thread = work / ((int64_t)kSampleThreads * 148 * 8);
    int items = kSamplerItemsMin;
    while (items < kSamplerItemsMax && items < per_thread) items *= 2;
    return items;
}
template <typename T> __host__ __device__ inline int tile_samples(int dim, int items)
{
    return (kSampleThreads * items) >> sampler_log2pad<T>(dim);
}


template <typename T, int kStore> __device__ __forceinline__ void store_block(T *row, const T *v, unsigned valid);
template <> __device__ __forceinline__ void store_block<float, 0>(float *row, const float *v, unsigned)
{
    *reinterpret_cast<float4 *>(row) = make_float4(v[0], v[1], v[2], v[3]);
}
template <> __device__ __forceinline__ void store_block<float, 1>(float *row, const float *v, unsigned valid)
{
    *reinterpret_cast<float2 *>(row) = make_float2(v[0], v[1]);
    if (valid & 4u) *reinterpret_cast<float2 *>(row + 2) = make_float2(v[2], v[3]);
}
template <> __device__ __forceinline__ void store_block<float, 2>(float *row, const float *v, unsigned valid)
{
#pragma unroll
    for (int k = 0; k < 4; ++k)
        if (valid & (1u << k)) row[k] = v[k];
}
template <> __device__ __forceinline__ void store_block<double, 0>(double *row, const double *v, unsigned)
{
    *reinterpret_cast<double2 *>(row) = make_double2(v[0], v[1]);
}
template <> __device__ __forceinline__ void store_block<double, 2>(double *row, const double *v, unsigned valid)
{
    row[0] = v[0];
    if (valid & 2u) row[1] = v[1];
}
template <> __device__ __forceinline__ void store_block<double, 1>(double *row, const double *v, unsigned valid)
{
    store_block<double, 2>(row, v, valid);
}

template <typename T, int kDrType, int kStore>
__global__ void __launch_bounds__(kSampleThreads) dr_sample_kernel(T *__restrict__ out, int64_t n, const DrCfgPrepared<T> cfg,
                                                                   uint64_t seed, uint64_t sample_id0, uint32_t call,
                                                                   unsigned long long *violations, int items)
{
    constexpr int P = Pack<T>::kPerBlock;
    const int dim = cfg.dim;
    const int kTile = tile_samples<T>(dim, items);
    const int blocks_per_sample = (dim + P - 1) / P;
    int log2pad = 0;
    while ((1 << log2pad) < blocks_per_sample) ++log2pad;
    const int j = threadIdx.x & ((1 << log2pad) - 1);
    const int lane_sample = threadIdx.x >> log2pad, samples_per_pass = kSampleThreads >> log2pad;
    const int64_t first = (int64_t)blockIdx.x * kTile;
    const int samples = (int)min((int64_t)kTile, n - first);
    if (j >= blocks_per_sample) return;
    const DimBlock<T> blk = load_dim_block(cfg, j);
    unsigned viol = 0;
    T *const tile = out + (first + lane_sample) * dim + j * P;
    const int row_step = samples_per_pass * dim;
    const uint64_t id0 = sample_id0 + (uint64_t)(first + lane_sample);
    int sidx = lane_sample, off = 0;
    for (; sidx < samples; sidx += samples_per_pass, off += row_step) {
        T v[P];
        const uint64_t id = id0 + (uint32_t)(sidx - lane_sample);
        const unsigned pending = first_attempt<T>(kDrType, blk, seed, id, call, kTasks, j, v);
        if (kDrType != kDrUniform && pending) viol += redraws<T>(kDrType, blk, seed, id, call, kTasks, j, pending, v);
        store_block<T, kStore>(tile + off, v, blk.valid);
    }
    if (kDrType == kDrGaussian && viol && violations) atomicAdd(violations, (unsigned long long)viol);
}

#ifndef RENV_SAMPLER_ILP
#define RENV_SAMPLER_ILP 2
#endif
constexpr int kSamplerIlp = RENV_SAMPLER_ILP;
#ifndef RENV_SAMPLER_F32_CTAS
#define RENV_SAMPLER_F32_CTAS 2
#endif
struct RedoneBlock { float v0, v1, v2, v3; unsigned viol; };
template <int kDrType>
__device__ __noinline__ RedoneBlock sampler_redo_block(const DrCfgPrepared<float> *cfg, uint64_t seed, uint64_t id,
                                                       uint32_t call, int j)
{
    const DimBlock<float> blk = load_dim_block(*cfg, j);
    float v[4];
    const unsigned pending = first_attempt<float>(kDrType, blk, seed, id, call, kTasks, j, v);
    const unsigned viol = pending ? redraws<float>(kDrType, blk, seed, id, call, kTasks, j, pending, v) : 0u;
    return RedoneBlock{ v[0], v[1], v[2], v[3], viol };
}

template <int kDrType, int kStore>
__global__ void __launch_bounds__(kSampleThreads, RENV_SAMPLER_F32_CTAS)
dr_sample_f32_kernel(float *__restrict__ out, int64_t n, const __grid_constant__ DrCfgPrepared<float> cfg, uint64_t seed,
                     const __grid_constant__ PhiloxKeys ks, uint64_t sample_id0, uint32_t call,
                     unsigned long long *violations, int items)
{
    const int dim = cfg.dim;
    const int kTile = tile_samples<float>(dim, items);
    const int blocks_per_sample = (dim + 3) / 4;
    int log2pad = 0;
    while ((1 << log2pad) < blocks_per_sample) ++log2pad;
    const int j = threadIdx.x & ((1 << log2pad) - 1);
    const int lane_sample = threadIdx.x >> log2pad, samples_per_pass = kSampleThreads >> log2pad;
    const int64_t first = (int64_t)blockIdx.x * kTile;
    const int samples = (int)min((int64_t)kTile, n - first);
    if (j >= blocks_per_sample || lane_sample >= samples) return;
    const DimBlockPacked pb = pack_dim_block(load_dim_block(cfg, j));
    unsigned viol = 0;
    float *row = out + (first + lane_sample) * dim + j * 4;
    const int64_t row_step = (int64_t)samples_per_pass * dim;
    const uint64_t id0 = sample_id0 + (uint64_t)(first + lane_sample);
    int todo = (samples - lane_sample + samples_per_pass - 1) / samples_per_pass;
    const uint64_t to_wrap = (0x100000000ull - (id0 & 0xffffffffull) + (uint64_t)samples_per_pass - 1) / (uint64_t)samples_per_pass;
    uint64_t id = id0;
    while (todo > 0) {
        const int seg = (int)min((uint64_t)todo, id == id0 ? to_wrap : (uint64_t)todo);
        const uint32_t c1 = (uint32_t)(id >> 32) & 0xffffu, c2 = call, c3 = ((uint32_t)kTasks << 24) | (uint32_t)j;
        uint32_t c0 = (uint32_t)id;
        auto one_block = [&](uint32_t ctr0, float *dst) {
            const uint4 r = philox4x32_10(make_uint4(ctr0, c1, c2, c3), ks);
            float v[4];
            if (first_attempt_packed<kDrType>(r, pb, v)) {
                const RedoneBlock b = sampler_redo_block<kDrType>(&cfg, seed, (id & ~0xffffffffull) | ctr0, call, j);
                v[0] = b.v0; v[1] = b.v1; v[2] = b.v2; v[3] = b.v3;
                viol += b.viol;
            }
            store_block<float, kStore>(dst, v, pb.valid);
        };
        int k = seg;
        if (kSamplerIlp == 2 && kDrType != kDrUniform) {
#pragma unroll 1
            for (; k >= 2; k -= 2) {
                const uint32_t c0b = c0 + (uint32_t)samples_per_pass;
                const uint4 ra = philox4x32_10(make_uint4(c0, c1, c2, c3), ks);
                const uint4 rb = philox4x32_10(make_uint4(c0b, c1, c2, c3), ks);
                float va[4], vb[4];
                const bool bad_a = first_attempt_packed<kDrType>(ra, pb, va);
                const bool bad_b = first_attempt_packed<kDrType>(rb, pb, vb);
                if (bad_a || bad_b) {
                    if (bad_a) {
                        const RedoneBlock b = sampler_redo_block<kDrType>(&cfg, seed, (id & ~0xffffffffull) | c0, call, j);
                        va[0] = b.v0; va[1] = b.v1; va[2] = b.v2; va[3] = b.v3;
                        viol += b.viol;
                    }
                    if (bad_b) {
                        const RedoneBlock b = sampler_redo_block<kDrType>(&cfg, seed, (id & ~0xffffffffull) | c0b, call, j);
                        vb[0] = b.v0; vb[1] = b.v1; vb[2] = b.v2; vb[3] = b.v3;
                        viol += b.viol;
                    }
                }
                store_block<float, kStore>(row, va, pb.valid);
                store_block<float, kStore>(row + row_step, vb, pb.valid);
                c0 += 2u * (uint32_t)samples_per_pass;
                row += 2 * row_step;
            }
        }
#pragma unroll 1
        for (; k > 0; --k) {
            one_block(c0, row);
            c0 += (uint32_t)samples_per_pass;
            row += row_step;
        }
        id += (uint64_t)seg * (uint64_t)samples_per_pass;
        todo -= seg;
    }
    if (kDrType == kDrGaussian && viol && violations) atomicAdd(violations, (unsigned long long)viol);
}

__device__ __forceinline__ double exact_u32_to_double(uint32_t v)
{
    return __dadd_rn(__hiloint2double(0x43300000, (int)v), -4503599627370496.0);
}
template <int kStore>
__global__ void __launch_bounds__(kSampleThreads, 3)
dr_sample_f64_uniform_kernel(double *__restrict__ out, int64_t n, const __grid_constant__ DrCfgPrepared<double> cfg,
                             const __grid_constant__ PhiloxKeys ks, uint64_t sample_id0, uint32_t call, int items)
{
    const int dim = cfg.dim;
    const int kTile = tile_samples<double>(dim, items);
    const int blocks_per_sample = (dim + 1) / 2;
    int log2pad = 0;
    while ((1 << log2pad) < blocks_per_sample) ++log2pad;
    const int j = threadIdx.x & ((1 << log2pad) - 1);
    const int lane_sample = threadIdx.x >> log2pad, samples_per_pass = kSampleThreads >> log2pad;
    const int64_t first = (int64_t)blockIdx.x * kTile;
    const int samples = (int)min((int64_t)kTile, n - first);
    if (j >= blocks_per_sample || lane_sample >= samples) return;
    const DimBlock<double> blk = load_dim_block(cfg, j);
    const double w0 = blk.b[0] * (1.0 / 9007199254740992.0), w1 = blk.b[1] * (1.0 / 9007199254740992.0);
    double *row = out + (first + lane_sample) * dim + j * 2;
    const int64_t row_step = (int64_t)samples_per_pass * dim;
    const uint64_t id0 = sample_id0 + (uint64_t)(first + lane_sample);
    int todo = (samples - lane_sample + samples_per_pass - 1) / samples_per_pass;
    const uint64_t to_wrap = (0x100000000ull - (id0 & 0xffffffffull) + (uint64_t)samples_per_pass - 1) / (uint64_t)samples_per_pass;
    uint64_t id = id0;
    while (todo > 0) {
        const int seg = (int)min((uint64_t)todo, id == id0 ? to_wrap : (uint64_t)todo);
        const uint32_t c1 = (uint32_t)(id >> 32) & 0xffffu, c2 = call, c3 = ((uint32_t)kTasks << 24) | (uint32_t)j;
        uint32_t c0 = (uint32_t)id;
#pragma unroll 1
        for (int k = seg; k > 0; --k) {
            const uint4 r = philox4x32_10(make_uint4(c0, c1, c2, c3), ks);
            const double m0 = fma(exact_u32_to_double(r.x >> 5), 67108864.0, exact_u32_to_double(r.y >> 6));
            const double m1 = fma(exact_u32_to_double(r.z >> 5), 67108864.0, exact_u32_to_double(r.w >> 6));
            double v[2] = { __dadd_rn(blk.a[0], __dmul_rn(w0, m0)), __dadd_rn(blk.a[1], __dmul_rn(w1, m1)) };
            store_block<double, kStore>(row, v, blk.valid);
            c0 += (uint32_t)samples_per_pass;
            row += row_step;
        }
        id += (uint64_t)seg * (uint64_t)samples_per_pass;
        todo -= seg;
    }
}

template <typename T> struct FullGaussCfg {
    int dim;
    T mean[32], lo[32], hi[32];
    T ft[32 * 32];
};
#ifndef RENV_FULLGAUSS_CTAS
#define RENV_FULLGAUSS_CTAS 4
#endif
constexpr int kFullGaussThreads = 128;

template <typename T, int D>
__global__ void __launch_bounds__(kFullGaussThreads, RENV_FULLGAUSS_CTAS)
dr_sample_fullgaussian_kernel(T *__restrict__ out, int64_t n, const __grid_constant__ FullGaussCfg<T> cfg, uint64_t seed,
                              uint64_t sample_id0, uint32_t call)
{
    constexpr int P = Pack<T>::kPerBlock;
    constexpr int W = 16 / (int)sizeof(T);
    __shared__ __align__(16) T stage[kFullGaussThreads * D];
    const int dim = cfg.dim;
    const int64_t i = (int64_t)blockIdx.x * kFullGaussThreads + threadIdx.x;
    const uint64_t id = sample_id0 + (uint64_t)i;
    T x[D];
#pragma unroll
    for (int d = 0; d < D; ++d) x[d] = cfg.mean[d];
    if (i < n) {
#pragma unroll
        for (int j = 0; j < D / P; ++j) {
            if (j * P < dim) {
                T z[P];
                Num<T>::normals(draw_block(seed, id, call, kTasks, (uint32_t)j), z);
#pragma unroll
                for (int kk = 0; kk < P; ++kk)
#pragma unroll
                    for (int d = 0; d < D; ++d)
                        x[d] = Num<T>::affine(cfg.ft[(j * P + kk) * 32 + d], z[kk], x[d]);
            }
        }
    }
    const int warp = threadIdx.x >> 5, lane = threadIdx.x & 31;
    T *tile = stage + warp * 32 * D;
#pragma unroll
    for (int d = 0; d < D; ++d)
        if (d < dim) tile[lane * dim + d] = denormalize(x[d], cfg.lo[d], cfg.hi[d]);
    __syncwarp();
    const int64_t warp_first = (int64_t)blockIdx.x * kFullGaussThreads + warp * 32;
    const int rows = (int)max((int64_t)0, min((int64_t)32, n - warp_first));
    const int total = rows * dim;
    T *dst = out + warp_first * dim;
    const int nvec = total / W;
    for (int q = lane; q < nvec; q += 32)
        reinterpret_cast<uint4 *>(dst)[q] = reinterpret_cast<const uint4 *>(tile)[q];
    for (int q = nvec * W + lane; q < total; q += 32) dst[q] = tile[q];
}

__global__ void __launch_bounds__(256) random_actions_kernel(uint8_t *__restrict__ action, int64_t n, uint64_t env_id0,
                                                             uint64_t seed, uint32_t step)
{
    const int64_t i0 = ((int64_t)blockIdx.x * blockDim.x + threadIdx.x) * 4;
    if (i0 >= n) return;
    uint32_t word = 0;
#pragma unroll
    for (int k = 0; k < 4; ++k) {
        const uint64_t e = env_id0 + (uint64_t)(i0 + k);
        const uint4 r = draw_block(seed, e, (uint64_t)(step >> 7), kAction, 0);
        word |= action_bit(r, step) << (8 * k);
    }
    if (i0 + 4 <= n) {
        *reinterpret_cast<uint32_t *>(action + i0) = word;
    } else {
        for (int k = 0; k < 4 && i0 + k < n; ++k) action[i0 + k] = (uint8_t)((word >> (8 * k)) & 1u);
    }
}

}
```

### random_envs_b200/csrc/renv_philox.cuh

```cuda
#pragma once
#include <stdint.h>

namespace renv {

enum Purpose : uint32_t { kInit = 0, kXi = 1, kAction = 2, kTasks = 3, kObs = 4, kPolicySample = 5 };

__device__ __forceinline__ uint4 philox4x32_10(uint4 c, uint2 k)
{
    constexpr uint32_t M0 = 0xD2511F53u, M1 = 0xCD9E8D57u, W0 = 0x9E3779B9u, W1 = 0xBB67AE85u;
#pragma unroll
    for (int r = 0; r < 10; ++r) {
        const uint32_t hi0 = __umulhi(M0, c.x), lo0 = M0 * c.x;
        const uint32_t hi1 = __umulhi(M1, c.z), lo1 = M1 * c.z;
        c = make_uint4(hi1 ^ c.y ^ k.x, lo1, hi0 ^ c.w ^ k.y, lo0);
        k.x += W0;
        k.y += W1;
    }
    return c;
}

struct PhiloxKeys { uint32_t x[10], y[10]; };
__host__ __device__ __forceinline__ PhiloxKeys philox_keys(uint32_t kx, uint32_t ky)
{
    constexpr uint32_t W0 = 0x9E3779B9u, W1 = 0xBB67AE85u;
    PhiloxKeys ks;
#pragma unroll
    for (int r = 0; r < 10; ++r) { ks.x[r] = kx + (uint32_t)r * W0; ks.y[r] = ky + (uint32_t)r * W1; }
    return ks;
}
__device__ __forceinline__ uint4 philox4x32_10(uint4 c, const PhiloxKeys &ks)
{
    constexpr uint32_t M0 = 0xD2511F53u, M1 = 0xCD9E8D57u;
#pragma unroll
    for (int r = 0; r < 10; ++r) {
        const uint32_t hi0 = __umulhi(M0, c.x), lo0 = M0 * c.x;
        const uint32_t hi1 = __umulhi(M1, c.z), lo1 = M1 * c.z;
        c = make_uint4(hi1 ^ c.y ^ ks.x[r], lo1, hi0 ^ c.w ^ ks.y[r], lo0);
    }
    return c;
}

__device__ __forceinline__ uint4 draw_block(uint64_t seed, uint64_t id, uint64_t tick, uint32_t purpose, uint32_t slot)
{
    const uint32_t c1 = ((uint32_t)(id >> 32) & 0xffffu) | (((uint32_t)(tick >> 32) & 0xffffu) << 16);
    return philox4x32_10(make_uint4((uint32_t)id, c1, (uint32_t)tick, (purpose << 24) | slot),
                         make_uint2((uint32_t)seed, (uint32_t)(seed >> 32)));
}

__device__ __forceinline__ float u01(uint32_t r) { return (float)(r >> 8) * (1.0f / 16777216.0f); }
__device__ __forceinline__ double u01(uint32_t hi, uint32_t lo)
{
    return __dmul_rn(__dadd_rn(__dmul_rn((double)(hi >> 5), 67108864.0), (double)(lo >> 6)),
                     1.0 / 9007199254740992.0);
}
__device__ __forceinline__ float u01_open0(uint32_t r) { return (float)((r >> 8) + 1u) * (1.0f / 16777216.0f); }
__device__ __forceinline__ double u01_open0(uint32_t hi, uint32_t lo)
{
    return __dmul_rn(__dadd_rn(__dadd_rn(__dmul_rn((double)(hi >> 5), 67108864.0), (double)(lo >> 6)), 1.0),
                     1.0 / 9007199254740992.0);
}

template <typename T> struct Pack;
template <> struct Pack<float> {
    static constexpr int kPerBlock = 4;
    __device__ static __forceinline__ void uniforms(uint4 r, float u[4])
    {
        u[0] = u01(r.x); u[1] = u01(r.y); u[2] = u01(r.z); u[3] = u01(r.w);
    }
    static constexpr float kUniformScale = 1.0f / 16777216.0f;
    __device__ static __forceinline__ float uniform_scale(float width) { return width * kUniformScale; }
    __device__ static __forceinline__ void uniform_affine(uint4 r, const float scale[4], const float off[4], float out[4])
    {
        out[0] = fmaf(scale[0], (float)(r.x >> 8), off[0]);
        out[1] = fmaf(scale[1], (float)(r.y >> 8), off[1]);
        out[2] = fmaf(scale[2], (float)(r.z >> 8), off[2]);
        out[3] = fmaf(scale[3], (float)(r.w >> 8), off[3]);
    }
    __device__ static __forceinline__ void normals(uint4 r, float z[4])
    {
        float s, c;
        float rad = sqrtf(-2.0f * logf(u01_open0(r.x)));
        sincospif(2.0f * u01(r.y), &s, &c);
        z[0] = rad * c; z[1] = rad * s;
        rad = sqrtf(-2.0f * logf(u01_open0(r.z)));
        sincospif(2.0f * u01(r.w), &s, &c);
        z[2] = rad * c; z[3] = rad * s;
    }
};
template <> struct Pack<double> {
    static constexpr int kPerBlock = 2;
    __device__ static __forceinline__ void uniforms(uint4 r, double u[2])
    {
        u[0] = u01(r.x, r.y); u[1] = u01(r.z, r.w);
    }
    __device__ static __forceinline__ double uniform_scale(double width) { return width; }
    __device__ static __forceinline__ void uniform_affine(uint4 r, const double scale[2], const double off[2], double out[2])
    {
        double u[2];
        uniforms(r, u);
        out[0] = __dadd_rn(off[0], __dmul_rn(scale[0], u[0]));
        out[1] = __dadd_rn(off[1], __dmul_rn(scale[1], u[1]));
    }
    __device__ static __forceinline__ void normals(uint4 r, double z[2])
    {
        double s, c;
        const double rad = sqrt(-2.0 * log(u01_open0(r.x, r.y)));
        sincospi(2.0 * u01(r.z, r.w), &s, &c);
        z[0] = rad * c; z[1] = rad * s;
    }
};

}
```

### random_envs_b200/csrc/renv_step_body.cuh

```cuda
    using VT = VecTraits<T>;
    constexpr int V = VT::V;
    constexpr int kTile = kStepThreads * V;
    __shared__ unsigned s_count;
    __shared__ uint16_t s_list[kAutoReset ? kTile : 1];
    __shared__ int32_t s_len[kLog ? kTile : 1];
    const int64_t block0 = (int64_t)blockIdx.x * kTile;
    const int64_t i0 = block0 + (int64_t)threadIdx.x * V;
    const int64_t n = a.env.n, ld = a.env.ld;
    const bool live = i0 < n;
    const bool full = i0 + V <= n;
    const bool tracked = a.env.progress != nullptr;
    uint32_t ticket = 0;

    if (tracked) {
        if (threadIdx.x == 0) {
            uint32_t *const slot = a.env.progress + 2 * (size_t)blockIdx.x;
            ticket = atomicAdd(slot, 1u);
            uint32_t seen = ld_acquire_gpu(slot + 1);
            for (int spin = 0; seen != ticket && spin < RENV_ORDER_SPINS; ++spin) {
                __nanosleep(32);
                seen = ld_acquire_gpu(slot + 1);
            }
            if (seen != ticket && a.counters) atomicAdd(a.counters + kCounterOrderTimeout, 1ull);
            if (kAutoReset) s_count = 0;
        } else if (RENV_TILE_PREFETCH && block0 + kTile <= n && threadIdx.x >= 32 && threadIdx.x < 39) {
            const int q = threadIdx.x - 32;
            if (q < 4) prefetch_l2(a.env.state + q * ld + block0, kTile * sizeof(T));
            else if (q == 4) prefetch_l2(a.env.xi + 4 * block0, kTile * 4 * sizeof(T));
            else if (q == 5) { if (kLean) prefetch_l2(a.env.elapsed16 + block0, kTile * 2); else prefetch_l2(a.env.elapsed + block0, kTile * 4); }
            else prefetch_l2(a.action + block0, kTile);
        }
        __syncthreads();
        asm volatile("griddepcontrol.launch_dependents;" ::: "memory");
    } else {
        asm volatile("griddepcontrol.wait;" ::: "memory");
    }

    T s[4][V];
    Xi<T> p[V];
    int32_t el[V];
    uint8_t act[V];
    if (full) {
#pragma unroll
        for (int c = 0; c < 4; ++c) vload<typename VT::Real>(s[c], a.env.state + c * ld + i0);
#pragma unroll
        for (int v = 0; v < V; ++v) p[v] = load_xi(a.env.xi, i0 + v);
        if (kLean) {
            uint16_t e16[V];
            vload<typename VT::Half>(e16, a.env.elapsed16 + i0);
#pragma unroll
            for (int v = 0; v < V; ++v) el[v] = e16[v];
        } else {
            vload<typename VT::Int>(el, a.env.elapsed + i0);
        }
        vload<typename VT::Byte>(act, a.action + i0);
    }
    if (kAutoReset && !tracked) {
        if (threadIdx.x == 0) s_count = 0;
        __syncthreads();
    }

    if (live) {
        if (!full) {
#pragma unroll
            for (int v = 0; v < V; ++v) {
                const bool ok = i0 + v < n;
#pragma unroll
                for (int c = 0; c < 4; ++c) s[c][v] = ok ? a.env.state[c * ld + i0 + v] : T(0);
                p[v] = ok ? load_xi(a.env.xi, i0 + v) : Xi<T>{ T(1), T(1), T(1), T(1) };
                el[v] = !ok ? 0 : kLean ? (int32_t)a.env.elapsed16[i0 + v] : a.env.elapsed[i0 + v];
                act[v] = ok ? a.action[i0 + v] : 0;
            }
        }

        T rew[V];
        uint8_t dn[V], tr[V];
        const bool euler = a.euler != 0;
        bool bad_action = false;
#pragma unroll
        for (int v = 0; v < V; ++v) {
            bad_action = bad_action || act[v] > 1;
            State<T> st = { s[0][v], s[1][v], s[2][v], s[3][v] };
            const bool terminated = dynamics(st, p[v], derive(p[v]), act[v], euler);
            s[0][v] = st.x; s[1][v] = st.x_dot; s[2][v] = st.theta; s[3][v] = st.theta_dot;
            el[v] += 1;
            bool done = terminated, trunc = false;
            if (a.max_steps > 0 && el[v] >= a.max_steps) { trunc = !terminated; done = true; }
            T r = T(1);
            if (!kAutoReset && i0 + v < n && terminated) {
                const int32_t b = a.env.beyond[i0 + v];
                a.env.beyond[i0 + v] = b < 0 ? 0 : b + 1;
                r = b < 0 ? T(1) : T(0);
            }
            rew[v] = r; dn[v] = done; tr[v] = trunc;
            if (kAutoReset && done && i0 + v < n) {
                const int32_t len = trunc ? -el[v] : el[v];
                el[v] = 0;
                if (kLog) {
                    const unsigned slot = atomicAdd(&s_count, 1u);
                    s_list[slot] = (uint16_t)(threadIdx.x * V + v);
                    s_len[slot] = len;
                } else {
                    s_list[atomicAdd(&s_count, 1u)] = (uint16_t)(threadIdx.x * V + v);
                }
            }
        }
        if (bad_action && a.counters) atomicAdd(a.counters + kCounterBadAction, 1ull);

        if (kNoisy) {
            T o[4][V];
#pragma unroll
            for (int v = 0; v < V; ++v) {
                T ov[4];
                add_obs_noise(State<T>{ s[0][v], s[1][v], s[2][v], s[3][v] }, a.env.noise_std, a.env.seed,
                              a.env.env_id0 + (uint64_t)(i0 + v), a.tick, 0u, ov);
#pragma unroll
                for (int c = 0; c < 4; ++c) o[c][v] = ov[c];
            }
            if (full) {
#pragma unroll
                for (int c = 0; c < 4; ++c) vstore<typename VT::Real>(a.env.obs + c * ld + i0, o[c]);
            } else {
#pragma unroll
                for (int v = 0; v < V; ++v)
                    if (i0 + v < n) {
#pragma unroll
                        for (int c = 0; c < 4; ++c) a.env.obs[c * ld + i0 + v] = o[c][v];
                    }
            }
        }

        if (!tracked) asm volatile("griddepcontrol.launch_dependents;" ::: "memory");
        if (full) {
#pragma unroll
            for (int c = 0; c < 4; ++c) vstore<typename VT::Real>(a.env.state + c * ld + i0, s[c]);
            if (kLean) {
                uint16_t e16[V];
#pragma unroll
                for (int v = 0; v < V; ++v) e16[v] = (uint16_t)el[v];
                vstore<typename VT::Half>(a.env.elapsed16 + i0, e16);
            } else {
                vstore<typename VT::Int>(a.env.elapsed + i0, el);
            }
            if (a.reward) vstore<typename VT::Real>(a.reward + i0, rew);
            vstore<typename VT::Byte>(a.done + i0, dn);
            if (a.truncated) vstore<typename VT::Byte>(a.truncated + i0, tr);
        } else {
#pragma unroll
            for (int v = 0; v < V; ++v) {
                if (i0 + v < n) {
#pragma unroll
                    for (int c = 0; c < 4; ++c) a.env.state[c * ld + i0 + v] = s[c][v];
                    if (kLean) a.env.elapsed16[i0 + v] = (uint16_t)el[v];
                    else a.env.elapsed[i0 + v] = el[v];
                    if (a.reward) a.reward[i0 + v] = rew[v];
                    a.done[i0 + v] = dn[v];
                    if (a.truncated) a.truncated[i0 + v] = tr[v];
                }
            }
        }
    } else if (!tracked) {
        asm volatile("griddepcontrol.launch_dependents;" ::: "memory");
    }

    if (kAutoReset) {
        __syncthreads();
        const unsigned count = s_count;
        unsigned viol = 0;
        for (unsigned j = threadIdx.x; j < count; j += kStepThreads) {
            if (kLog) {
                const int64_t i = block0 + s_list[j];
                const int32_t len = s_len[j];
                const State<T> fs = { a.env.state[i], a.env.state[ld + i], a.env.state[2 * ld + i], a.env.state[3 * ld + i] };
                const uint32_t c = (uint32_t)log.count[i];
                log_episode(log, ld, i, c, load_xi(a.env.xi, i), fs, len < 0 ? -len : len, len < 0, a.tick);
                log.count[i] = (int32_t)(c + 1u);
            }
            viol += reset_env(a.env, a.dr, block0 + s_list[j], a.tick, a.env.seed);
        }
        if (viol && a.counters) atomicAdd(a.counters + kCounterGaussian, (unsigned long long)viol);
    }
    if (tracked) {
        __syncthreads();
        if (threadIdx.x == 0) {
            st_release_gpu(a.env.progress + 2 * (size_t)blockIdx.x + 1, ticket + 1u);
            asm volatile("griddepcontrol.wait;" ::: "memory");
        }
    }
```

### random_envs_b200/vector_env.py

```python
import ctypes
import math

import numpy as np

from . import _device, _lib
from .episode_log import EpisodeLog
from .mlp_policy import MLPPolicy
from .random_env import RandomEnv
from .trajectory import Trajectory
from .xi_tables import get_table

_TABLE = get_table("RandomCartPole-v0")
NOMINAL_TASK = (9.8, 1.0, 0.1, 0.5)
THETA_THRESHOLD_RADIANS = 12 * 2 * math.pi / 360
X_THRESHOLD = 2.4
MAX_EPISODE_STEPS = 500


def _round_up(x, m):
    return (x + m - 1) // m * m


class RandomCartPoleVecEnv(RandomEnv):

    def __init__(self, num_envs, dtype="float32", device=None, seed=0, env_id0=0,
                 max_episode_steps=MAX_EPISODE_STEPS, auto_reset=True, kinematics_integrator="euler",
                 track_truncated=True, validate_actions=True, track_episodes=True, noisy=False, noise_level=1e-4,
                 lean=False, tile_ordering="auto", pack_host_flags=True):
        RandomEnv.__init__(self)
        if num_envs <= 0:
            raise ValueError("num_envs must be positive")
        self.num_envs = int(num_envs)
        self.pack_host_flags = bool(pack_host_flags)
        self._dtype_name = str(dtype).replace("torch.", "")
        if self._dtype_name not in ("float32", "float64"):
            raise ValueError("dtype must be float32 or float64")
        self._device_arg = device
        self._seed = int(seed) & 0xFFFFFFFFFFFFFFFF
        self.env_id0 = int(env_id0)
        self.max_episode_steps = 0 if max_episode_steps is None else int(max_episode_steps)
        self.auto_reset = bool(auto_reset)
        self.kinematics_integrator = kinematics_integrator
        self.track_truncated = bool(track_truncated)
        self.validate_actions = bool(validate_actions)
        self.track_episodes = bool(track_episodes)
        self.noisy = bool(noisy)
        self.noise_level = float(noise_level)
        if self.noise_level < 0:
            raise ValueError("noise_level must be >= 0")
        self.lean = bool(lean)
        if self.lean and (self._dtype_name != "float32" or not self.auto_reset or self.noisy
                          or not 0 < self.max_episode_steps <= 65535):
            raise ValueError("lean=True needs float32, auto_reset, no observation noise and 0 < max_episode_steps <= 65535")

        self.tile_ordering = (self.num_envs <= (1 << 21)) if tile_ordering == "auto" else bool(tile_ordering)

        self.dyn_ind_to_name = dict(enumerate(_TABLE.names))
        self.original_task = np.array(NOMINAL_TASK)
        self.task_dim = 4
        self.min_task = np.zeros(4)
        self.max_task = np.zeros(4)
        self.mean_task = np.zeros(4)
        self.stdev_task = np.zeros(4)
        self.reward_threshold = _TABLE.reward_threshold
        self.theta_threshold_radians = THETA_THRESHOLD_RADIANS
        self.x_threshold = X_THRESHOLD
        self.force_mag, self.tau = 10.0, 0.02
        self.polemass_length = 0.05
        self._buffers = None
        self._episode_log = None
        self._cfg_cache = None
        self._cfg_key = None
        self._tick = 0
        self.seed_dr(self._seed)

    def get_search_bounds_mean(self, index):
        return _TABLE.search_bounds[index]

    def get_task_lower_bound(self, index):
        return _TABLE.lower_bounds[index]

    @property
    def torch_dtype(self):
        t = _device.torch()
        return t.float32 if self._dtype_name == "float32" else t.float64

    @property
    def device(self):
        return self._alloc()["device"]

    def _alloc(self):
        if self._buffers is not None:
            return self._buffers
        t = _device.torch()
        dev = _device.require_cuda(self._device_arg)
        _lib.load()
        n, ld = self.num_envs, _round_up(self.num_envs, 32)
        dt = self.torch_dtype
        b = dict(device=dev, ld=ld)
        b["state"] = t.zeros((4, ld), dtype=dt, device=dev)
        b["xi"] = t.tensor(NOMINAL_TASK, dtype=dt, device=dev).reshape(1, 4).repeat(ld, 1).contiguous()
        b["elapsed"] = None if self.lean else t.zeros(ld, dtype=t.int32, device=dev)
        b["elapsed16"] = t.zeros(ld, dtype=t.int16, device=dev) if self.lean else None
        b["episode"] = t.zeros(ld, dtype=t.int32, device=dev)
        b["beyond"] = t.full((ld,), -1, dtype=t.int32, device=dev)
        b["reward"] = t.ones(ld, dtype=dt, device=dev)
        b["done"] = t.zeros(ld, dtype=t.uint8, device=dev)
        b["truncated"] = t.zeros(ld, dtype=t.uint8, device=dev)
        b["action"] = t.zeros(ld, dtype=t.uint8, device=dev)
        b["stats"] = t.tensor([0.0, 0.0, 0.0, math.inf, -math.inf, 0.0], dtype=t.float64, device=dev)
        b["obs"] = t.zeros((4, ld), dtype=dt, device=dev) if self.noisy else None
        tiles = -(-n // _lib.TILE_ENVS[self._dtype_name])
        b["progress"] = t.zeros(2 * tiles, dtype=t.int32, device=dev) if self.tile_ordering else None
        b["env"] = None
        self._buffers = b
        self._refresh_env_struct()
        return b

    def _refresh_env_struct(self):
        b = self._buffers
        env = _lib.CartpoleEnv()
        env.state, env.xi = b["state"].data_ptr(), b["xi"].data_ptr()
        env.elapsed = None if self.lean else b["elapsed"].data_ptr()
        env.elapsed16 = b["elapsed16"].data_ptr() if self.lean else None
        env.beyond = b["beyond"].data_ptr()
        env.progress = b["progress"].data_ptr() if b["progress"] is not None else None
        env.episode = b["episode"].data_ptr() if self.track_episodes else None
        env.n, env.ld = self.num_envs, b["ld"]
        env.env_id0, env.seed = self.env_id0, self._seed
        b["env"] = env
        b["step_plan"] = None
        b["noise"] = None
        if self.noisy:
            b["noise"] = _lib.ObsNoise()
            b["noise"].obs, b["noise"].std = b["obs"].data_ptr(), math.sqrt(self.noise_level)

    def _entry(self, name):
        b = self._buffers
        if self._episode_log is not None and name in ("step", "rollout"):
            return "renv_cartpole_%s_logged_%s" % (name, self._suffix()), (ctypes.byref(b["env"]),
                                                                          ctypes.byref(self._episode_log.struct))
        if self.noisy:
            b["noise"].std = math.sqrt(self.noise_level)
            return "renv_cartpole_%s_noisy_%s" % (name, self._suffix()), (ctypes.byref(b["env"]), ctypes.byref(b["noise"]))
        return "renv_cartpole_%s_%s" % (name, self._suffix()), (ctypes.byref(b["env"]),)

    def _suffix(self):
        return "f32" if self._dtype_name == "float32" else "f64"

    def _integrator(self):
        return _lib.EULER if self.kinematics_integrator == "euler" else _lib.SEMI_IMPLICIT

    def _on_distribution_change(self):
        self._cfg_cache = None

    def _active_dr_cfg(self):
        if not self.dr_training or self.sampling is None:
            return None
        key = (self.sampling, self.min_task.tobytes(), self.max_task.tobytes(), self.mean_task.tobytes(),
               self.stdev_task.tobytes(),
               np.asarray(self.cov_task).tobytes() if self.sampling == "fullgaussian" else None)
        if self._cfg_cache is None or self._cfg_key != key:
            self._cfg_cache, self._cfg_key = self.dr_config(), key
        return ctypes.byref(self._cfg_cache)

    def seed(self, seed=None):
        if seed is None:
            seed = int(np.random.SeedSequence().entropy % (2 ** 63))
        self._seed = int(seed) & 0xFFFFFFFFFFFFFFFF
        self.seed_dr(self._seed)
        self._tick = 0
        if self._buffers is not None:
            self._refresh_env_struct()
        return [seed]

    def reset(self, mask=None):
        b = self._alloc()
        t = _device.torch()
        mask_ptr = None
        if mask is not None:
            mask = t.as_tensor(mask, device=b["device"]).to(t.uint8).contiguous()
            assert mask.shape == (self.num_envs,)
            mask_ptr = _device.ptr(mask)
        viol = self._violation_counter(b["device"])
        fn, head = self._entry("reset")
        with t.cuda.device(b["device"]):
            _lib.call(fn, *head, mask_ptr, self._tick,
                      self._active_dr_cfg(), _device.ptr(viol), _device.stream_ptr(b["device"]))
        self._tick += 1
        return self.obs

    @property
    def obs(self):
        b = self._alloc()
        return (b["obs"] if self.noisy else b["state"])[:, :self.num_envs].t()

    @property
    def state(self):
        return self._alloc()["state"][:, :self.num_envs].t()

    def _stage_actions(self, actions):
        b = self._buffers
        t = _device.torch()
        n = self.num_envs
        if isinstance(actions, t.Tensor) and actions.is_cuda and actions.dtype == t.uint8 and actions.is_contiguous() \
                and actions.data_ptr() % 16 == 0 and actions.device == b["device"] \
                and (tuple(actions.shape) == (n,) or actions is b["action"]):
            return actions
        src = actions if isinstance(actions, t.Tensor) else t.as_tensor(np.asarray(actions))
        if tuple(src.shape) != (n,):
            raise ValueError("actions must have shape (%d,), got %s" % (n, tuple(src.shape)))
        if src.dtype.is_floating_point:
            raise AssertionError("%r (%s) invalid" % (actions, type(actions)))
        if src.dtype == t.bool:
            src = src.to(t.uint8)
        elif src.dtype != t.uint8:
            src = src.to(b["device"], non_blocking=True)
            src = t.where((src < 0) | (src > 255), t.full_like(src, 255), src)
        b["action"][:n].copy_(src, non_blocking=True)
        return b["action"]

    def _step_plan(self):
        b = self._buffers
        key = (self.noisy, self.track_truncated, self._dtype_name, self.lean, self._episode_log, self.auto_reset)
        plan = b.get("step_plan")
        if plan is not None and plan["key"] == key:
            return plan
        t = _device.torch()
        n = self.num_envs
        if self._episode_log is not None:
            self._check_log_supported()
        fn, head = self._entry("step_lean" if self.lean else "step")
        info = {"TimeLimit.truncated": b["truncated"][:n].view(t.bool)} if self.track_truncated else {}
        viol = self._violation_counter(b["device"])
        plan = dict(key=key, fn=getattr(_lib.load(), fn), name=fn, head=head, logged=self._episode_log is not None,
                    reward=_device.ptr(b["reward"]), done=_device.ptr(b["done"]),
                    truncated=_device.ptr(b["truncated"]) if self.track_truncated else None,
                    out=(self.obs, b["reward"][:n], b["done"][:n].view(t.bool)), info=info,
                    device_index=b["device"].index, viol=ctypes.c_void_p(viol.data_ptr()), viol_tensor=viol,
                    own_action=b["action"], own_action_ptr=_device.ptr(b["action"]))
        b["step_plan"] = plan
        return plan

    def step(self, actions):
        b = self._alloc()
        t = _device.torch()
        plan = self._step_plan()
        if actions is plan["own_action"] or actions is b.get("action_view"):
            action_ptr = plan["own_action_ptr"]
        else:
            action_ptr = ctypes.c_void_p(self._stage_actions(actions).data_ptr())
        if self.noisy:
            b["noise"].std = math.sqrt(self.noise_level)
        idx = plan["device_index"]
        if self.lean:
            args = plan["head"] + (action_ptr, plan["done"], plan["truncated"], self._integrator(), self.max_episode_steps,
                                   self._tick, self._active_dr_cfg(), plan["viol"], ctypes.c_void_p(_device.raw_stream(idx)))
        elif plan["logged"]:
            args = plan["head"] + (action_ptr, plan["reward"], plan["done"], plan["truncated"],
                                   self._integrator(), self.max_episode_steps, self._tick,
                                   self._active_dr_cfg(), plan["viol"], ctypes.c_void_p(_device.raw_stream(idx)))
        else:
            args = plan["head"] + (action_ptr, plan["reward"], plan["done"], plan["truncated"],
                                   self._integrator(), self.max_episode_steps, int(self.auto_reset), self._tick,
                                   self._active_dr_cfg(), plan["viol"], ctypes.c_void_p(_device.raw_stream(idx)))
        if t.cuda.current_device() == idx:
            rc = plan["fn"](*args)
        else:
            with t.cuda.device(b["device"]):
                rc = plan["fn"](*args)
        if rc != _lib.OK:
            raise _lib.RenvError(plan["name"], rc, _lib.strerror(rc))
        self._tick += 1
        obs, reward, done = plan["out"]
        return obs, reward, done, dict(plan["info"])

    def _own_action_view(self):
        b = self._buffers
        v = b.get("action_view")
        if v is None:
            v = b["action_view"] = b["action"][:self.num_envs]
        return v

    def sample_actions(self, out=None):
        b = self._alloc()
        t = _device.torch()
        out = b["action"] if out is None else out
        with t.cuda.device(b["device"]):
            _lib.call("renv_random_actions_u8", _device.ptr(out), self.num_envs, self.env_id0, self._seed,
                      self._tick & 0xFFFFFFFF, _device.stream_ptr(b["device"]))
        return self._own_action_view() if out is b["action"] else out

    def _check_mlp_supported(self, policy, what):
        if not isinstance(policy, MLPPolicy):
            raise TypeError("%s takes an MLPPolicy (MLPPolicy.from_module(net, device))" % what)
        if self._dtype_name != "float32" or self.noisy:
            raise ValueError("%s with an MLPPolicy needs a float32 env without observation noise" % what)
        if policy.device != self._alloc()["device"]:
            raise ValueError("the MLPPolicy lives on %s, the env on %s" % (policy.device, self._buffers["device"]))

    def policy_actions(self, policy, return_logits=False, *, sample=False, return_logp=False):
        self._check_mlp_supported(policy, "policy_actions()")
        b = self._buffers
        t = _device.torch()
        n = self.num_envs
        logits = logp = None
        if return_logits:
            logits = b.get("mlp_logits")
            if logits is None:
                logits = b["mlp_logits"] = t.empty((2, b["ld"]), dtype=t.float32, device=b["device"])
        if return_logp:
            logp = b.get("mlp_logp")
            if logp is None:
                logp = b["mlp_logp"] = t.empty(b["ld"], dtype=t.float32, device=b["device"])
        with t.cuda.device(b["device"]):
            if sample or return_logp:
                _lib.call("renv_cartpole_policy_logp_mlp_f32", ctypes.byref(b["env"]), ctypes.byref(policy.struct),
                          int(bool(sample)), self._tick, _device.ptr(b["action"]), _device.ptr(logp), _device.ptr(logits),
                          _device.stream_ptr(b["device"]))
            else:
                _lib.call("renv_cartpole_policy_actions_mlp_f32", ctypes.byref(b["env"]), ctypes.byref(policy.struct),
                          _device.ptr(b["action"]), _device.ptr(logits), _device.stream_ptr(b["device"]))
        out = (self._own_action_view(),) + ((logits[:, :n].t(),) if return_logits else ()) + \
            ((logp[:n],) if return_logp else ())
        return out if len(out) > 1 else out[0]

    def trajectory_buffer(self, capacity, logp=True, final_obs=True):
        b = self._alloc()
        return Trajectory(self.num_envs, b["ld"], capacity, b["device"], logp=logp, final_obs=final_obs)

    def collect(self, policy, num_steps, sample=True, out=None):
        buf = self._alloc()
        t = _device.torch()
        if self.lean:
            raise ValueError("collect() keeps the int32 TimeLimit counter: build the env without lean=True")
        self._check_mlp_supported(policy, "collect()")
        K = int(num_steps)
        if K < 1:
            raise ValueError("num_steps must be >= 1, got %d" % K)
        if out is None:
            out = self.trajectory_buffer(K)
        elif not isinstance(out, Trajectory) or out.num_envs != self.num_envs or out.ld != buf["ld"] \
                or out.device != buf["device"]:
            raise ValueError("out is not a trajectory buffer of this env's shape and device: use trajectory_buffer()")
        elif out.capacity < K:
            raise ValueError("out holds %d steps, collect() was asked for %d" % (out.capacity, K))
        head = (ctypes.byref(buf["env"]),)
        fn = "renv_cartpole_collect_mlp_f32"
        if self._episode_log is not None:
            self._check_log_supported()
            fn, head = "renv_cartpole_collect_mlp_logged_f32", head + (ctypes.byref(self._episode_log.struct),)
        viol = self._violation_counter(buf["device"])
        with t.cuda.device(buf["device"]):
            _lib.call(fn, *head, ctypes.byref(policy.struct), ctypes.byref(out.struct), int(bool(sample)), K,
                      self._integrator(), self.max_episode_steps, self._tick, self._active_dr_cfg(),
                      _device.ptr(buf["stats"]), _device.ptr(viol), _device.stream_ptr(buf["device"]))
        out.tick0, out.num_steps = self._tick, K
        self._tick += K
        return out

    def _rollout_mlp(self, policy, b, num_steps):
        self._check_mlp_supported(policy, "rollout()")
        if float(b) != 0.0:
            raise ValueError("an MLPPolicy carries its own biases: rollout(policy) takes no b")
        buf = self._buffers
        t = _device.torch()
        head = (ctypes.byref(buf["env"]),)
        fn = "renv_cartpole_rollout_mlp_f32"
        if self._episode_log is not None:
            self._check_log_supported()
            fn, head = "renv_cartpole_rollout_mlp_logged_f32", head + (ctypes.byref(self._episode_log.struct),)
        viol = self._violation_counter(buf["device"])
        with t.cuda.device(buf["device"]):
            _lib.call(fn, *head, ctypes.byref(policy.struct), int(num_steps), self._integrator(), self.max_episode_steps,
                      self._tick, self._active_dr_cfg(), _device.ptr(buf["stats"]), _device.ptr(viol),
                      _device.stream_ptr(buf["device"]))
        self._tick += int(num_steps)

    def rollout(self, w, b=0.0, num_steps=MAX_EPISODE_STEPS):
        buf = self._alloc()
        t = _device.torch()
        if self.lean:
            raise ValueError("rollout() keeps the int32 TimeLimit counter: build the env without lean=True")
        if isinstance(w, MLPPolicy):
            return self._rollout_mlp(w, b, num_steps)
        if w is None:
            if self.noisy:
                raise ValueError("the random policy ignores observations: use a noise-free env")
            w_arr = None
        else:
            w_arr = (ctypes.c_double * 4)(*[float(v) for v in w])
        if self._episode_log is not None:
            self._check_log_supported()
        viol = self._violation_counter(buf["device"])
        fn, head = self._entry("rollout")
        with t.cuda.device(buf["device"]):
            _lib.call(fn, *head, w_arr, float(b),
                      int(num_steps), self._integrator(), self.max_episode_steps, self._tick, self._active_dr_cfg(),
                      _device.ptr(buf["stats"]), _device.ptr(viol), _device.stream_ptr(buf["device"]))
        self._tick += int(num_steps)

    def start_episode_log(self, capacity=1):
        self._check_log_supported()
        b = self._alloc()
        self._episode_log = EpisodeLog(self.num_envs, b["ld"], capacity, self.torch_dtype, b["device"], self.env_id0)
        return self._episode_log

    def stop_episode_log(self):
        if self._episode_log is None:
            self._check_log_supported()
        self._episode_log = None

    def _check_log_supported(self):
        if self.lean or self.noisy or not self.auto_reset:
            raise ValueError("the episode log needs an auto-reset env without lean=True or observation noise")

    @property
    def episode_log(self):
        return self._episode_log

    @property
    def stats_tensor(self):
        return self._alloc()["stats"]

    def reset_stats(self):
        t = _device.torch()
        self._alloc()["stats"].copy_(t.tensor([0.0, 0.0, 0.0, math.inf, -math.inf, 0.0], dtype=t.float64))

    def allgather_stats(self, group=None):
        from .distributed import allgather_stats
        combined, gathered = allgather_stats(self.stats_tensor, group)
        host = combined.cpu()
        self.check_dr_violations()
        return host, gathered

    def episode_stats(self):
        from .distributed import summarize_stats
        stats = self.stats_tensor.cpu().numpy()
        self.check_dr_violations()
        return summarize_stats(stats)

    def check_dr_violations(self):
        if not self.validate_actions and self._dr_violations is not None:
            self._dr_violations[_lib.COUNTER_BAD_ACTION] = 0
        RandomEnv.check_dr_violations(self)

    def get_task(self):
        return self._alloc()["xi"][:self.num_envs]

    def set_task(self, *task):
        b = self._alloc()
        t = _device.torch()
        n = self.num_envs
        if len(task) == 1:
            xi = t.as_tensor(task[0], device=b["device"]).to(self.torch_dtype)
            if xi.shape == (4,):
                xi = xi.reshape(1, 4).expand(n, 4)
            if xi.shape != (n, 4):
                raise ValueError("set_task expects (N, 4) or 4 scalars")
            b["xi"][:n].copy_(xi)
        elif len(task) == 4:
            b["xi"][:n].copy_(t.tensor([float(v) for v in task], dtype=self.torch_dtype,
                                       device=b["device"]).reshape(1, 4).expand(n, 4))
        else:
            raise ValueError("set_task expects (N, 4) or 4 scalars")

    def set_random_task(self):
        self.set_task(self.sample_tasks_tensor(self.num_envs, dtype=self.torch_dtype, device=self._alloc()["device"],
                                               sample_id0=self.env_id0))
        self.check_dr_violations()

    def host_buffers(self):
        b = self._alloc()
        t = _device.torch()
        n = self.num_envs
        h = b.get("host")
        if h is None:
            h = dict(action=t.empty(b["ld"], dtype=t.uint8).pin_memory(),
                     state=t.empty((4, b["ld"]), dtype=self.torch_dtype).pin_memory(),
                     reward=t.empty(b["ld"], dtype=self.torch_dtype).pin_memory(),
                     done=t.empty(b["ld"], dtype=t.uint8).pin_memory(),
                     truncated=t.empty(b["ld"], dtype=t.uint8).pin_memory(),
                     counters=t.zeros(_lib.NUM_COUNTERS, dtype=t.int64).pin_memory())
            words = (b["ld"] + 31) // 32
            h["flag_bits"] = t.zeros((2, words), dtype=t.int32).pin_memory()
            b["flag_bits"] = t.zeros((2, words), dtype=t.int32, device=b["device"])
            h["flag_bytes"] = h["flag_bits"].numpy().view(np.uint8)
            h["np"] = dict(action=h["action"].numpy()[:n], obs=h["state"].numpy()[:, :n].T,
                           reward=h["reward"].numpy()[:n], done=h["done"].numpy()[:n].view(np.bool_),
                           truncated=h["truncated"].numpy()[:n].view(np.bool_))
            h["reward"].fill_(1)
            h["stream"] = t.cuda.Stream(device=b["device"])
            h["event"] = t.cuda.Event()
            b["host"] = h
        return h["np"]

    def step_host_async(self, actions=None):
        views = self.host_buffers()
        b = self._buffers
        h = b["host"]
        t = _device.torch()
        if actions is not None:
            acts = np.asarray(actions)
            if acts.dtype != np.uint8:
                if acts.dtype.kind not in "iu":
                    raise AssertionError("%r (%s) invalid" % (actions, type(actions)))
                acts = np.clip(acts, -1, 2)
            np.copyto(views["action"], acts, casting="unsafe")
        stream = h["stream"]
        stream.wait_stream(t.cuda.current_stream(b["device"]))
        with t.cuda.stream(stream):
            b["action"].copy_(h["action"], non_blocking=True)
            self.step(b["action"])
            h["state"].copy_(b["obs"] if self.noisy else b["state"], non_blocking=True)
            if not self.auto_reset:
                h["reward"].copy_(b["reward"], non_blocking=True)
            if self.pack_host_flags:
                sp = _device.stream_ptr(b["device"])
                bits = b["flag_bits"]
                _lib.call("renv_pack_flags_u8", _device.ptr(b["done"]), _device.ptr(bits[0]), self.num_envs, sp)
                if self.track_truncated:
                    _lib.call("renv_pack_flags_u8", _device.ptr(b["truncated"]), _device.ptr(bits[1]), self.num_envs, sp)
                    h["flag_bits"].copy_(bits, non_blocking=True)
                else:
                    h["flag_bits"][0].copy_(bits[0], non_blocking=True)
            else:
                h["done"].copy_(b["done"], non_blocking=True)
                if self.track_truncated:
                    h["truncated"].copy_(b["truncated"], non_blocking=True)
            h["counters"].copy_(self._violation_counter(b["device"]), non_blocking=True)
            h["event"].record(stream)

    def host_bytes_per_step(self):
        esize = 4 if self._dtype_name == "float32" else 8
        ld = self._alloc()["ld"]
        flag = 4 * ((ld + 31) // 32) if self.pack_host_flags else ld
        d2h = 4 * ld * esize + flag + (0 if self.auto_reset else ld * esize) + (flag if self.track_truncated else 0) \
            + 8 * _lib.NUM_COUNTERS
        return ld, d2h

    def step_host_wait(self):
        h = self._buffers["host"]
        h["event"].synchronize()
        c = h["counters"]
        if int(c[0]) | int(c[1]):
            self.check_dr_violations()
        v = h["np"]
        if self.pack_host_flags:
            n = self.num_envs
            np.copyto(v["done"].view(np.uint8), np.unpackbits(h["flag_bytes"][0], count=n, bitorder="little"))
            if self.track_truncated:
                np.copyto(v["truncated"].view(np.uint8), np.unpackbits(h["flag_bytes"][1], count=n, bitorder="little"))
        return v["obs"], v["reward"], v["done"], v["truncated"]

    def step_host(self, actions):
        self.step_host_async(actions)
        return self.step_host_wait()

    def _tensor_keys(self):
        return ("state", "xi", "elapsed16" if self.lean else "elapsed", "episode", "beyond", "stats") + \
               (("obs",) if self.noisy else ())

    def state_dict(self):
        b = self._alloc()
        out = {k: b[k].clone() for k in self._tensor_keys()}
        out.update(seed=self._seed, env_id0=self.env_id0, tick=self._tick, num_envs=self.num_envs,
                   dtype=self._dtype_name, lean=self.lean,
                   dr=dict(seed=self._dr_seed, calls=self._dr_calls, sampling=self.sampling, dr_training=self.dr_training,
                           min_task=self.min_task.copy(), max_task=self.max_task.copy(), mean_task=self.mean_task.copy(),
                           stdev_task=self.stdev_task.copy(),
                           cov_task=np.copy(self.cov_task) if getattr(self, "cov_task", None) is not None else None))
        self.check_dr_violations()
        return out

    def load_state_dict(self, sd):
        if sd["num_envs"] != self.num_envs or sd["dtype"] != self._dtype_name or sd.get("lean", False) != self.lean:
            raise ValueError("state_dict is for %d %s envs%s" % (sd["num_envs"], sd["dtype"], " (lean)" if sd.get("lean") else ""))
        b = self._alloc()
        for k in self._tensor_keys():
            b[k].copy_(sd[k])
        self._seed, self.env_id0, self._tick = sd["seed"], sd["env_id0"], sd["tick"]
        dr = sd.get("dr")
        if dr is not None:
            self._dr_seed, self._dr_calls = dr["seed"], dr["calls"]
            self.sampling, self.dr_training = dr["sampling"], dr["dr_training"]
            self.min_task[:], self.max_task[:] = dr["min_task"], dr["max_task"]
            self.mean_task[:], self.stdev_task[:] = dr["mean_task"], dr["stdev_task"]
            if dr["cov_task"] is not None:
                self.cov_task = np.copy(dr["cov_task"])
            self._on_distribution_change()
        self._refresh_env_struct()

    @property
    def elapsed(self):
        b = self._alloc()
        if self.lean:
            t = _device.torch()
            return b["elapsed16"][:self.num_envs].to(t.int32) & 0xFFFF
        return b["elapsed"][:self.num_envs]

    @property
    def episode(self):
        return self._alloc()["episode"][:self.num_envs]

    @property
    def steps_beyond_done(self):
        return self._alloc()["beyond"][:self.num_envs]

    def set_state(self, state, elapsed=None):
        b = self._alloc()
        t = _device.torch()
        st = t.as_tensor(state, device=b["device"]).to(self.torch_dtype)
        b["state"][:, :self.num_envs].copy_(st.t())
        b["beyond"].fill_(-1)
        if elapsed is not None:
            el = t.as_tensor(elapsed, device=b["device"]).to(t.int32)
            if self.lean:
                b["elapsed16"][:self.num_envs].copy_(el.to(t.int16))
            else:
                b["elapsed"][:self.num_envs].copy_(el)
```

Before: 92.38 billion.

## Regenerate uniform DR parameters from episode start tick instead of storing xi

Adds a regen step kernel that recomputes each env's uniform-DR task parameters from Philox using a stored 32-bit episode start tick, instead of reading and writing the 4-float xi array every step. A materialize kernel rebuilds xi on demand for get_task/state_dict, and Python-side bookkeeping falls back to stored mode for noisy, lean, logged, tile-ordered or non-uniform cases. This trades per-step HBM traffic for extra Philox arithmetic and adds state-tracking complexity.

```diff
diff --git a/include/renv.h b/include/renv.h
--- a/include/renv.h
+++ b/include/renv.h
@@ -91,6 +91,12 @@
 int renv_cartpole_step_lean_f32(const renv_cartpole_env *env, const uint8_t *action, uint8_t *done, uint8_t *truncated,
                                 int integrator, int max_steps, uint64_t tick, const renv_dr_cfg *dr,
                                 unsigned long long *counters, void *stream);
+
+int renv_cartpole_step_regen_f32(const renv_cartpole_env *env, uint32_t *start_tick, const uint8_t *action, float *reward,
+                                 uint8_t *done, uint8_t *truncated, int integrator, int max_steps, int auto_reset,
+                                 uint64_t tick, const renv_dr_cfg *dr, unsigned long long *counters, void *stream);
+int renv_cartpole_materialize_xi_f32(const renv_cartpole_env *env, const uint32_t *start_tick, uint64_t tick,
+                                     const renv_dr_cfg *dr, void *stream);
 
 typedef struct renv_obs_noise {
     void *obs;
diff --git a/profiles/time_step_xi.py b/profiles/time_step_xi.py
--- /dev/null
+++ b/profiles/time_step_xi.py
@@ -0,0 +1,146 @@
+import argparse
+import json
+import os
+import subprocess
+import sys
+
+ROOT = os.path.dirname(os.path.dirname(os.path.abspath(__file__)))
+sys.path.insert(0, ROOT)
+
+import torch
+
+import random_envs_b200 as renv
+from random_envs_b200 import _device, _lib
+
+SEARCH = [2.0, 20.0, 0.5, 3.0, 0.05, 0.3, 0.1, 1.0]
+BYTES = {"stored": 62, "regen": 50}
+CASES = [
+    ("branches_4x2^20", 1 << 20, 4, True, False, False),
+    ("single_2^24", 1 << 24, 1, False, False, False),
+    ("single_2^26", 1 << 26, 1, False, False, False),
+]
+
+
+def gpu_info():
+    info = dict(gpu=torch.cuda.get_device_name(0))
+    try:
+        q = subprocess.run(["nvidia-smi", "--query-gpu=power.limit,clocks.max.sm", "--format=csv,noheader"],
+                           capture_output=True, text=True, timeout=30).stdout.strip().splitlines()
+        info["power_limit_and_max_sm_clock"] = q[0] if q else "unknown"
+    except (OSError, subprocess.SubprocessError) as exc:
+        info["power_limit_and_max_sm_clock"] = "unknown (%s)" % exc
+    return info
+
+
+def peak_gbs():
+    try:
+        with open(os.path.join(ROOT, "MEASURED_PEAKS.json")) as f:
+            return float(json.load(f)["hbm_gbs"])
+    except (OSError, ValueError, KeyError):
+        return None
+
+
+def make_batches(n, R, tile_ordering, lean, mode, dev):
+    envs, actions = [], []
+    for b in range(R):
+        env = renv.RandomCartPoleVecEnv(n, device=dev, seed=0, env_id0=b * n, track_truncated=False,
+                                        track_episodes=False, tile_ordering=tile_ordering, lean=lean)
+        env._xi_mode = "auto" if mode == "regen" else "stored"
+        env.set_dr_distribution("uniform", SEARCH)
+        env.set_dr_training(True)
+        env.reset()
+        acts = []
+        for k in range(8):
+            a = torch.empty(n, dtype=torch.uint8, device=dev)
+            _lib.call("renv_random_actions_u8", _device.ptr(a), n, env.env_id0, 0, k, _device.stream_ptr(dev))
+            acts.append(a)
+        envs.append(env)
+        actions.append(acts)
+    return envs, actions
+
+
+def capture(envs, actions, K, parallel, dev):
+    R = len(envs)
+    for i in range(2 * R):
+        envs[i % R].step(actions[i % R][0])
+    torch.cuda.synchronize()
+    g = torch.cuda.CUDAGraph()
+    side = torch.cuda.Stream(device=dev)
+    side.wait_stream(torch.cuda.current_stream())
+    with torch.cuda.stream(side):
+        with torch.cuda.graph(g, stream=side):
+            if parallel:
+                lanes = [torch.cuda.Stream(device=dev) for _ in range(R)]
+                for b, lane in enumerate(lanes):
+                    lane.wait_stream(side)
+                    with torch.cuda.stream(lane):
+                        for i in range(b, K, R):
+                            envs[b].step(actions[b][(i // R) % 8])
+                for lane in lanes:
+                    side.wait_stream(lane)
+            else:
+                for i in range(K):
+                    envs[i % R].step(actions[i % R][(i // R) % 8])
+    torch.cuda.current_stream().wait_stream(side)
+    return g
+
+
+def time_graph(g):
+    e0, e1 = torch.cuda.Event(enable_timing=True), torch.cuda.Event(enable_timing=True)
+    torch.cuda.synchronize()
+    g.replay()
+    e0.record()
+    g.replay()
+    e1.record()
+    torch.cuda.synchronize()
+    return e0.elapsed_time(e1)
+
+
+def main():
+    ap = argparse.ArgumentParser()
+    ap.add_argument("--out", default=None)
+    ap.add_argument("--rounds", type=int, default=3)
+    ap.add_argument("--steps", type=int, default=200)
+    args = ap.parse_args()
+    dev = torch.device("cuda", 0)
+    renv.load_library()
+    peak = peak_gbs()
+    result = dict(info=gpu_info(), steps=args.steps, rounds=args.rounds, peak_gbs=peak, cases={})
+    for name, n, R, parallel, tiles, lean in CASES:
+        K = args.steps - args.steps % R
+        graphs, keep = {}, []
+        for mode in ("stored", "regen"):
+            envs, actions = make_batches(n, R, tiles, lean, mode, dev)
+            graphs[mode] = capture(envs, actions, K, parallel, dev)
+            expect = "renv_cartpole_step_regen_f32" if mode == "regen" else "renv_cartpole_step_f32"
+            assert envs[0]._buffers["step_plan"]["name"] == expect, envs[0]._buffers["step_plan"]["name"]
+            keep.append((envs, actions))
+        us = {"stored": [], "regen": []}
+        for _ in range(args.rounds):
+            for mode in ("stored", "regen"):
+                us[mode].append(1e3 * time_graph(graphs[mode]) / K)
+        case = {}
+        for mode, v in us.items():
+            v = sorted(v)
+            b = BYTES[mode]
+            best = v[0]
+            gbs = b * n / (best * 1e-6) / 1e9
+            case[mode] = dict(us_per_launch=v, best_us=best, median_us=v[len(v) // 2], spread=v[-1] / v[0] - 1,
+                              bytes_per_env_step=b, gbs_at_best=gbs, frac_of_peak=gbs / peak if peak else None)
+        case["speedup_median"] = case["stored"]["median_us"] / case["regen"]["median_us"]
+        result["cases"][name] = case
+        print("%-20s stored %7.2f us  regen %7.2f us  x%.3f" % (name, case["stored"]["median_us"],
+                                                               case["regen"]["median_us"], case["speedup_median"]),
+              file=sys.stderr)
+        del graphs, keep
+        torch.cuda.empty_cache()
+    text = json.dumps(result, indent=1)
+    if args.out:
+        os.makedirs(os.path.dirname(os.path.abspath(args.out)), exist_ok=True)
+        with open(args.out, "w") as f:
+            f.write(text + "\n")
+    print(text)
+
+
+if __name__ == "__main__":
+    main()
diff --git a/random_envs_b200/_lib.py b/random_envs_b200/_lib.py
--- a/random_envs_b200/_lib.py
+++ b/random_envs_b200/_lib.py
@@ -70,6 +70,8 @@
     "renv_cartpole_step_f32": (_int, [_env_p, _vp, _vp, _vp, _vp, _int, _int, _int, _u64, _cfg_p, _vp, _vp]),
     "renv_cartpole_step_f64": (_int, [_env_p, _vp, _vp, _vp, _vp, _int, _int, _int, _u64, _cfg_p, _vp, _vp]),
     "renv_cartpole_step_lean_f32": (_int, [_env_p, _vp, _vp, _vp, _int, _int, _u64, _cfg_p, _vp, _vp]),
+    "renv_cartpole_step_regen_f32": (_int, [_env_p, _vp, _vp, _vp, _vp, _vp, _int, _int, _int, _u64, _cfg_p, _vp, _vp]),
+    "renv_cartpole_materialize_xi_f32": (_int, [_env_p, _vp, _u64, _cfg_p, _vp]),
     "renv_cartpole_reset_noisy_f32": (_int, [_env_p, _noise_p, _vp, _u64, _cfg_p, _vp, _vp]),
     "renv_cartpole_reset_noisy_f64": (_int, [_env_p, _noise_p, _vp, _u64, _cfg_p, _vp, _vp]),
     "renv_cartpole_step_noisy_f32": (_int, [_env_p, _noise_p, _vp, _vp, _vp, _vp, _int, _int, _int, _u64, _cfg_p, _vp, _vp]),
diff --git a/random_envs_b200/csrc/renv_abi.cu b/random_envs_b200/csrc/renv_abi.cu
--- a/random_envs_b200/csrc/renv_abi.cu
+++ b/random_envs_b200/csrc/renv_abi.cu
@@ -261,12 +261,41 @@
     return launch_status();
 }
 
+int materialize_xi(const renv_cartpole_env *env, const uint32_t *start_tick, uint64_t tick, const renv_dr_cfg *dr,
+                   void *stream)
+{
+    MaterializeArgs a;
+    int rc = check_env<float>(env, false, &a.env, kNeedEitherElapsed);
+    if (rc) return rc;
+    if (start_tick == nullptr) return RENV_E_NULL;
+    if ((rc = to_cfg4<float>(dr, &a.dr))) return rc;
+    if (a.dr.dr_type != kDrUniform) return RENV_E_DRTYPE;
+    a.start_tick = start_tick;
+    a.tick = tick;
+    a.ks = philox_keys((uint32_t)env->seed, (uint32_t)(env->seed >> 32));
+    const int64_t blocks = (env->n + 255) / 256;
+    if (blocks > 0x7fffffffLL) return RENV_E_SIZE;
+    cartpole_materialize_xi_kernel<<<(unsigned)blocks, 256, 0, static_cast<cudaStream_t>(stream)>>>(a);
+    return launch_status();
+}
+
+int launch_step_regen(const StepArgs<float> &a, uint32_t *start_tick, unsigned blocks, cudaStream_t st)
+{
+    RegenStepArgs r;
+    r.step = a;
+    r.regen.start_tick = start_tick;
+    r.regen.ks = philox_keys((uint32_t)a.env.seed, (uint32_t)(a.env.seed >> 32));
+    return launch_pdl(cartpole_step_regen_kernel, blocks, kStepThreads, st, r);
+}
+int launch_step_regen(const StepArgs<double> &, uint32_t *, unsigned, cudaStream_t) { return RENV_E_ARG; }
+
 template <typename T, bool kLean>
 int cartpole_step(const renv_cartpole_env *env, const renv_obs_noise *noise, const uint8_t *action, T *reward,
                   uint8_t *done, uint8_t *truncated, int integrator, int max_steps, int auto_reset, uint64_t tick,
                   const renv_dr_cfg *dr, unsigned long long *counters, void *stream,
-                  const renv_episode_log *log = nullptr, bool logged = false)
-{
+                  const renv_episode_log *log = nullptr, bool logged = false, uint32_t *start_tick = nullptr)
+{
+    const bool regen = start_tick != nullptr;
     StepArgs<T> a;
     int rc = check_env<T>(env, !auto_reset, &a.env, kLean ? kNeedElapsed16 : kNeedElapsed32);
     if (rc) return rc;
@@ -283,6 +312,8 @@
     if (kLean && max_steps > 65535) return RENV_E_SIZE;
     rc = to_cfg4<T>(auto_reset ? dr : nullptr, &a.dr);
     if (rc) return rc;
+    if (regen && !aligned(start_tick, 16)) return RENV_E_ALIGN;
+    if (regen && a.dr.dr_type != kDrUniform) return auto_reset ? RENV_E_DRTYPE : RENV_E_ARG;
     a.action = action; a.reward = reward; a.done = done; a.truncated = truncated;
     a.euler = integrator == RENV_EULER;
     a.max_steps = max_steps;
@@ -297,6 +328,7 @@
         la.step = a;
         return launch_pdl(cartpole_step_logged_kernel<T>, (unsigned)blocks, kStepThreads, st, la);
     }
+    if (regen) return launch_step_regen(a, start_tick, (unsigned)blocks, st);
     if (kLean) return launch_pdl(cartpole_step_kernel<T, true, false, true>, (unsigned)blocks, kStepThreads, st, a);
     if (auto_reset && !noisy) return launch_pdl(cartpole_step_kernel<T, true, false>, (unsigned)blocks, kStepThreads, st, a);
     if (auto_reset) return launch_pdl(cartpole_step_kernel<T, true, true>, (unsigned)blocks, kStepThreads, st, a);
@@ -626,6 +658,19 @@
     return cartpole_step<float, true>(env, nullptr, action, nullptr, done, truncated, integrator, max_steps, 1, tick, dr,
                                       counters, stream);
 }
+int renv_cartpole_step_regen_f32(const renv_cartpole_env *env, uint32_t *start_tick, const uint8_t *action, float *reward,
+                                 uint8_t *done, uint8_t *truncated, int integrator, int max_steps, int auto_reset,
+                                 uint64_t tick, const renv_dr_cfg *dr, unsigned long long *counters, void *stream)
+{
+    if (start_tick == nullptr) return RENV_E_NULL;
+    return cartpole_step<float, false>(env, nullptr, action, reward, done, truncated, integrator, max_steps, auto_reset,
+                                       tick, dr, counters, stream, nullptr, false, start_tick);
+}
+int renv_cartpole_materialize_xi_f32(const renv_cartpole_env *env, const uint32_t *start_tick, uint64_t tick,
+                                     const renv_dr_cfg *dr, void *stream)
+{
+    return materialize_xi(env, start_tick, tick, dr, stream);
+}
 int renv_cartpole_step_f64(const renv_cartpole_env *env, const uint8_t *action, double *reward, uint8_t *done,
                            uint8_t *truncated, int integrator, int max_steps, int auto_reset, uint64_t tick,
                            const renv_dr_cfg *dr, unsigned long long *violations, void *stream)
diff --git a/random_envs_b200/csrc/renv_cartpole.cuh b/random_envs_b200/csrc/renv_cartpole.cuh
--- a/random_envs_b200/csrc/renv_cartpole.cuh
+++ b/random_envs_b200/csrc/renv_cartpole.cuh
@@ -243,4 +243,15 @@
     return violations;
 }
 
-}
+__device__ __forceinline__ Xi<float> uniform_xi(const DrCfg4<float> &cfg, const PhiloxKeys &ks, uint64_t id, uint64_t tick)
+{
+    float v[4];
+    Pack<float>::uniform_affine(draw_block(ks, id, tick, kXi, 0), cfg.b, cfg.a, v);
+    return Xi<float>{ v[0], v[1], v[2], v[3] };
+}
+__device__ __forceinline__ uint64_t episode_tick(uint64_t tick, uint32_t start_lo)
+{
+    return tick + (uint64_t)(int64_t)(int32_t)(start_lo - (uint32_t)tick);
+}
+
+}
diff --git a/random_envs_b200/csrc/renv_kernels.cuh b/random_envs_b200/csrc/renv_kernels.cuh
--- a/random_envs_b200/csrc/renv_kernels.cuh
+++ b/random_envs_b200/csrc/renv_kernels.cuh
@@ -61,7 +61,7 @@
     T *obs; T noise_std;
 };
 
-template <typename T>
+template <typename T, bool kRegenXi = false>
 __device__ __forceinline__ unsigned reset_env(const EnvPtrs<T> &env, const DrCfg4<T> &dr, int64_t i, uint64_t tick, uint64_t seed)
 {
     const int64_t ld = env.ld;
@@ -76,7 +76,7 @@
         env.obs[0 * ld + i] = o[0]; env.obs[1 * ld + i] = o[1]; env.obs[2 * ld + i] = o[2]; env.obs[3 * ld + i] = o[3];
     }
     unsigned viol = 0;
-    if (dr.dr_type != kDrNone) {
+    if (!kRegenXi && dr.dr_type != kDrNone) {
         Xi<T> xi = { T(0), T(0), T(0), T(0) };
         viol = sample_xi(xi, dr, seed, id, tick);
         store_xi(env.xi, i, xi);
@@ -138,6 +138,10 @@
     DrCfg4<T> dr;
     unsigned long long *counters;
 };
+struct RegenStepExtra {
+    uint32_t *start_tick;
+    PhiloxKeys ks;
+};
 
 #ifndef RENV_STEP_THREADS
 #define RENV_STEP_THREADS 256
@@ -150,20 +154,44 @@
 template <typename T, bool kAutoReset, bool kNoisy = false, bool kLean = false>
 __global__ void __launch_bounds__(kStepThreads, kNoisy ? (sizeof(T) == 8 ? 2 : 3) : RENV_STEP_MIN_CTAS(T)) cartpole_step_kernel(const __grid_constant__ StepArgs<T> a)
 {
-    constexpr bool kLog = false;
+    constexpr bool kLog = false, kRegenXi = false;
+    const LogPtrs<T> log = {};
+    const RegenStepExtra regen = {};
+#include "renv_step_body.cuh"
+}
+
+template <typename T> struct LoggedStepArgs { StepArgs<T> step; LogPtrs<T> log; };
+
+template <typename T>
+__global__ void __launch_bounds__(kStepThreads, RENV_STEP_MIN_CTAS(T)) cartpole_step_logged_kernel(const __grid_constant__ LoggedStepArgs<T> args)
+{
+    constexpr bool kAutoReset = true, kNoisy = false, kLean = false, kLog = true, kRegenXi = false;
+    const StepArgs<T> &a = args.step;
+    const LogPtrs<T> &log = args.log;
+    const RegenStepExtra regen = {};
+#include "renv_step_body.cuh"
+}
+
+#ifndef RENV_STEP_REGEN_CTAS
+#define RENV_STEP_REGEN_CTAS 3
+#endif
+struct RegenStepArgs { StepArgs<float> step; RegenStepExtra regen; };
+__global__ void __launch_bounds__(kStepThreads, RENV_STEP_REGEN_CTAS) cartpole_step_regen_kernel(const __grid_constant__ RegenStepArgs args)
+{
+    using T = float;
+    constexpr bool kAutoReset = true, kNoisy = false, kLean = false, kLog = false, kRegenXi = true;
+    const StepArgs<T> &a = args.step;
+    const RegenStepExtra &regen = args.regen;
     const LogPtrs<T> log = {};
 #include "renv_step_body.cuh"
 }
 
-template <typename T> struct LoggedStepArgs { StepArgs<T> step; LogPtrs<T> log; };
-
-template <typename T>
-__global__ void __launch_bounds__(kStepThreads, RENV_STEP_MIN_CTAS(T)) cartpole_step_logged_kernel(const __grid_constant__ LoggedStepArgs<T> args)
-{
-    constexpr bool kAutoReset = true, kNoisy = false, kLean = false, kLog = true;
-    const StepArgs<T> &a = args.step;
-    const LogPtrs<T> &log = args.log;
-#include "renv_step_body.cuh"
+struct MaterializeArgs { EnvPtrs<float> env; const uint32_t *start_tick; uint64_t tick; DrCfg4<float> dr; PhiloxKeys ks; };
+__global__ void __launch_bounds__(256) cartpole_materialize_xi_kernel(const __grid_constant__ MaterializeArgs a)
+{
+    const int64_t i = (int64_t)blockIdx.x * blockDim.x + threadIdx.x;
+    if (i >= a.env.n) return;
+    store_xi(a.env.xi, i, uniform_xi(a.dr, a.ks, a.env.env_id0 + (uint64_t)i, episode_tick(a.tick, a.start_tick[i])));
 }
 
 template <typename T> struct ResetArgs {
diff --git a/random_envs_b200/csrc/renv_philox.cuh b/random_envs_b200/csrc/renv_philox.cuh
--- a/random_envs_b200/csrc/renv_philox.cuh
+++ b/random_envs_b200/csrc/renv_philox.cuh
@@ -45,6 +45,11 @@
     const uint32_t c1 = ((uint32_t)(id >> 32) & 0xffffu) | (((uint32_t)(tick >> 32) & 0xffffu) << 16);
     return philox4x32_10(make_uint4((uint32_t)id, c1, (uint32_t)tick, (purpose << 24) | slot),
                          make_uint2((uint32_t)seed, (uint32_t)(seed >> 32)));
+}
+__device__ __forceinline__ uint4 draw_block(const PhiloxKeys &ks, uint64_t id, uint64_t tick, uint32_t purpose, uint32_t slot)
+{
+    const uint32_t c1 = ((uint32_t)(id >> 32) & 0xffffu) | (((uint32_t)(tick >> 32) & 0xffffu) << 16);
+    return philox4x32_10(make_uint4((uint32_t)id, c1, (uint32_t)tick, (purpose << 24) | slot), ks);
 }
 
 __device__ __forceinline__ float u01(uint32_t r) { return (float)(r >> 8) * (1.0f / 16777216.0f); }
diff --git a/random_envs_b200/csrc/renv_step_body.cuh b/random_envs_b200/csrc/renv_step_body.cuh
--- a/random_envs_b200/csrc/renv_step_body.cuh
+++ b/random_envs_b200/csrc/renv_step_body.cuh
@@ -26,7 +26,7 @@
         } else if (RENV_TILE_PREFETCH && block0 + kTile <= n && threadIdx.x >= 32 && threadIdx.x < 39) {
             const int q = threadIdx.x - 32;
             if (q < 4) prefetch_l2(a.env.state + q * ld + block0, kTile * sizeof(T));
-            else if (q == 4) prefetch_l2(a.env.xi + 4 * block0, kTile * 4 * sizeof(T));
+            else if (q == 4) { if (kRegenXi) prefetch_l2(regen.start_tick + block0, kTile * 4); else prefetch_l2(a.env.xi + 4 * block0, kTile * 4 * sizeof(T)); }
             else if (q == 5) { if (kLean) prefetch_l2(a.env.elapsed16 + block0, kTile * 2); else prefetch_l2(a.env.elapsed + block0, kTile * 4); }
             else prefetch_l2(a.action + block0, kTile);
         }
@@ -40,7 +40,21 @@
     Xi<T> p[V];
     int32_t el[V];
     uint8_t act[V];
-    if (full) {
+    int32_t start[V];
+    if (full && kRegenXi) {
+        vload<typename VT::Int>(start, reinterpret_cast<const int32_t *>(regen.start_tick) + i0);
+        if (kLean) {
+            uint16_t e16[V];
+            vload<typename VT::Half>(e16, a.env.elapsed16 + i0);
+#pragma unroll
+            for (int v = 0; v < V; ++v) el[v] = e16[v];
+        } else {
+            vload<typename VT::Int>(el, a.env.elapsed + i0);
+        }
+#pragma unroll
+        for (int c = 0; c < 4; ++c) vload<typename VT::Real>(s[c], a.env.state + c * ld + i0);
+        vload<typename VT::Byte>(act, a.action + i0);
+    } else if (full) {
 #pragma unroll
         for (int c = 0; c < 4; ++c) vload<typename VT::Real>(s[c], a.env.state + c * ld + i0);
 #pragma unroll
@@ -67,7 +81,8 @@
                 const bool ok = i0 + v < n;
 #pragma unroll
                 for (int c = 0; c < 4; ++c) s[c][v] = ok ? a.env.state[c * ld + i0 + v] : T(0);
-                p[v] = ok ? load_xi(a.env.xi, i0 + v) : Xi<T>{ T(1), T(1), T(1), T(1) };
+                if (!kRegenXi) p[v] = ok ? load_xi(a.env.xi, i0 + v) : Xi<T>{ T(1), T(1), T(1), T(1) };
+                else start[v] = ok ? (int32_t)regen.start_tick[i0 + v] : 0;
                 el[v] = !ok ? 0 : kLean ? (int32_t)a.env.elapsed16[i0 + v] : a.env.elapsed[i0 + v];
                 act[v] = ok ? a.action[i0 + v] : 0;
             }
@@ -81,6 +96,8 @@
         for (int v = 0; v < V; ++v) {
             bad_action = bad_action || act[v] > 1;
             State<T> st = { s[0][v], s[1][v], s[2][v], s[3][v] };
+            if constexpr (kRegenXi)
+                p[v] = uniform_xi(a.dr, regen.ks, a.env.env_id0 + (uint64_t)(i0 + v), episode_tick(a.tick, (uint32_t)start[v]));
             const bool terminated = dynamics(st, p[v], derive(p[v]), act[v], euler);
             s[0][v] = st.x; s[1][v] = st.x_dot; s[2][v] = st.theta; s[3][v] = st.theta_dot;
             el[v] += 1;
@@ -176,7 +193,8 @@
                 log_episode(log, ld, i, c, load_xi(a.env.xi, i), fs, len < 0 ? -len : len, len < 0, a.tick);
                 log.count[i] = (int32_t)(c + 1u);
             }
-            viol += reset_env(a.env, a.dr, block0 + s_list[j], a.tick, a.env.seed);
+            viol += reset_env<T, kRegenXi>(a.env, a.dr, block0 + s_list[j], a.tick, a.env.seed);
+            if (kRegenXi) regen.start_tick[block0 + s_list[j]] = (uint32_t)a.tick;
         }
         if (viol && a.counters) atomicAdd(a.counters + kCounterGaussian, (unsigned long long)viol);
     }
diff --git a/random_envs_b200/vector_env.py b/random_envs_b200/vector_env.py
--- a/random_envs_b200/vector_env.py
+++ b/random_envs_b200/vector_env.py
@@ -72,6 +72,9 @@
         self._cfg_cache = None
         self._cfg_key = None
         self._tick = 0
+        self._xi_mode = "auto"
+        self._xi_regen = self._xi_stale = False
+        self._xi_cfg = self._xi_key = None
         self.seed_dr(self._seed)
 
     def get_search_bounds_mean(self, index):
@@ -112,6 +115,8 @@
         b["obs"] = t.zeros((4, ld), dtype=dt, device=dev) if self.noisy else None
         tiles = -(-n // _lib.TILE_ENVS[self._dtype_name])
         b["progress"] = t.zeros(2 * tiles, dtype=t.int32, device=dev) if self.tile_ordering else None
+        regen_ok = self._dtype_name == "float32" and not self.lean and not self.tile_ordering
+        b["start_tick"] = t.zeros(ld, dtype=t.int32, device=dev) if regen_ok else None
         b["env"] = None
         self._buffers = b
         self._refresh_env_struct()
@@ -152,21 +157,45 @@
         return _lib.EULER if self.kinematics_integrator == "euler" else _lib.SEMI_IMPLICIT
 
     def _on_distribution_change(self):
+        self._xi_break()
         self._cfg_cache = None
+
+    def set_dr_training(self, flag):
+        self._xi_break()
+        RandomEnv.set_dr_training(self, flag)
+
+    def _materialize_xi(self):
+        if not self._xi_stale:
+            return
+        b = self._buffers
+        t = _device.torch()
+        with t.cuda.device(b["device"]):
+            _lib.call("renv_cartpole_materialize_xi_f32", ctypes.byref(b["env"]), _device.ptr(b["start_tick"]),
+                      self._tick, ctypes.byref(self._xi_cfg), _device.stream_ptr(b["device"]))
+        self._xi_stale = False
+
+    def _xi_break(self):
+        if self._xi_regen:
+            self._materialize_xi()
+            self._xi_regen = False
 
     def _active_dr_cfg(self):
         if not self.dr_training or self.sampling is None:
+            self._xi_break()
             return None
         key = (self.sampling, self.min_task.tobytes(), self.max_task.tobytes(), self.mean_task.tobytes(),
                self.stdev_task.tobytes(),
                np.asarray(self.cov_task).tobytes() if self.sampling == "fullgaussian" else None)
         if self._cfg_cache is None or self._cfg_key != key:
+            if key != self._xi_key:
+                self._xi_break()
             self._cfg_cache, self._cfg_key = self.dr_config(), key
         return ctypes.byref(self._cfg_cache)
 
     def seed(self, seed=None):
         if seed is None:
             seed = int(np.random.SeedSequence().entropy % (2 ** 63))
+        self._xi_break()
         self._seed = int(seed) & 0xFFFFFFFFFFFFFFFF
         self.seed_dr(self._seed)
         self._tick = 0
@@ -184,9 +213,21 @@
             mask_ptr = _device.ptr(mask)
         viol = self._violation_counter(b["device"])
         fn, head = self._entry("reset")
+        if mask is not None:
+            self._xi_break()
+        cfg = self._active_dr_cfg()
         with t.cuda.device(b["device"]):
-            _lib.call(fn, *head, mask_ptr, self._tick,
-                      self._active_dr_cfg(), _device.ptr(viol), _device.stream_ptr(b["device"]))
+            _lib.call(fn, *head, mask_ptr, self._tick, cfg, _device.ptr(viol), _device.stream_ptr(b["device"]))
+            if mask is None:
+                self._xi_stale = False
+                self._xi_regen = (self._xi_mode == "auto" and cfg is not None and self._dtype_name == "float32"
+                                  and not self.noisy and b["start_tick"] is not None
+                                  and self._cfg_cache.dr_type == _lib.DR_UNIFORM)
+                if self._xi_regen:
+                    lo = self._tick & 0xFFFFFFFF
+                    b["start_tick"].fill_(lo - (1 << 32) if lo >= 1 << 31 else lo)
+                    self._xi_cfg = _lib.DrCfg.from_buffer_copy(self._cfg_cache)
+                    self._xi_key = self._cfg_key
         self._tick += 1
         return self.obs
 
@@ -222,7 +263,8 @@
 
     def _step_plan(self):
         b = self._buffers
-        key = (self.noisy, self.track_truncated, self._dtype_name, self.lean, self._episode_log, self.auto_reset)
+        key = (self.noisy, self.track_truncated, self._dtype_name, self.lean, self._episode_log, self.auto_reset,
+               self._xi_regen, self._xi_mode)
         plan = b.get("step_plan")
         if plan is not None and plan["key"] == key:
             return plan
@@ -230,10 +272,19 @@
         n = self.num_envs
         if self._episode_log is not None:
             self._check_log_supported()
+        regen = self._xi_regen and self._xi_mode == "auto" and self.auto_reset and not self.noisy \
+            and self._episode_log is None and not self.lean and not self.tile_ordering
+        if self._xi_regen and not regen:
+            self._xi_break()
+            return self._step_plan()
         fn, head = self._entry("step_lean" if self.lean else "step")
+        if regen:
+            fn = "renv_cartpole_step_regen_f32"
+            head = head + (_device.ptr(b["start_tick"]),)
         info = {"TimeLimit.truncated": b["truncated"][:n].view(t.bool)} if self.track_truncated else {}
         viol = self._violation_counter(b["device"])
         plan = dict(key=key, fn=getattr(_lib.load(), fn), name=fn, head=head, logged=self._episode_log is not None,
+                    regen=regen,
                     reward=_device.ptr(b["reward"]), done=_device.ptr(b["done"]),
                     truncated=_device.ptr(b["truncated"]) if self.track_truncated else None,
                     out=(self.obs, b["reward"][:n], b["done"][:n].view(t.bool)), info=info,
@@ -245,6 +296,7 @@
     def step(self, actions):
         b = self._alloc()
         t = _device.torch()
+        cfg = self._active_dr_cfg()
         plan = self._step_plan()
         if actions is plan["own_action"] or actions is b.get("action_view"):
             action_ptr = plan["own_action_ptr"]
@@ -255,15 +307,15 @@
         idx = plan["device_index"]
         if self.lean:
             args = plan["head"] + (action_ptr, plan["done"], plan["truncated"], self._integrator(), self.max_episode_steps,
-                                   self._tick, self._active_dr_cfg(), plan["viol"], ctypes.c_void_p(_device.raw_stream(idx)))
+                                   self._tick, cfg, plan["viol"], ctypes.c_void_p(_device.raw_stream(idx)))
         elif plan["logged"]:
             args = plan["head"] + (action_ptr, plan["reward"], plan["done"], plan["truncated"],
                                    self._integrator(), self.max_episode_steps, self._tick,
-                                   self._active_dr_cfg(), plan["viol"], ctypes.c_void_p(_device.raw_stream(idx)))
+                                   cfg, plan["viol"], ctypes.c_void_p(_device.raw_stream(idx)))
         else:
             args = plan["head"] + (action_ptr, plan["reward"], plan["done"], plan["truncated"],
                                    self._integrator(), self.max_episode_steps, int(self.auto_reset), self._tick,
-                                   self._active_dr_cfg(), plan["viol"], ctypes.c_void_p(_device.raw_stream(idx)))
+                                   cfg, plan["viol"], ctypes.c_void_p(_device.raw_stream(idx)))
         if t.cuda.current_device() == idx:
             rc = plan["fn"](*args)
         else:
@@ -271,6 +323,7 @@
                 rc = plan["fn"](*args)
         if rc != _lib.OK:
             raise _lib.RenvError(plan["name"], rc, _lib.strerror(rc))
+        self._xi_stale = self._xi_stale or plan["regen"]
         self._tick += 1
         obs, reward, done = plan["out"]
         return obs, reward, done, dict(plan["info"])
@@ -345,6 +398,7 @@
             raise ValueError("out is not a trajectory buffer of this env's shape and device: use trajectory_buffer()")
         elif out.capacity < K:
             raise ValueError("out holds %d steps, collect() was asked for %d" % (out.capacity, K))
+        self._xi_break()
         head = (ctypes.byref(buf["env"]),)
         fn = "renv_cartpole_collect_mlp_f32"
         if self._episode_log is not None:
@@ -365,6 +419,7 @@
             raise ValueError("an MLPPolicy carries its own biases: rollout(policy) takes no b")
         buf = self._buffers
         t = _device.torch()
+        self._xi_break()
         head = (ctypes.byref(buf["env"]),)
         fn = "renv_cartpole_rollout_mlp_f32"
         if self._episode_log is not None:
@@ -392,6 +447,7 @@
             w_arr = (ctypes.c_double * 4)(*[float(v) for v in w])
         if self._episode_log is not None:
             self._check_log_supported()
+        self._xi_break()
         viol = self._violation_counter(buf["device"])
         fn, head = self._entry("rollout")
         with t.cuda.device(buf["device"]):
@@ -403,6 +459,7 @@
     def start_episode_log(self, capacity=1):
         self._check_log_supported()
         b = self._alloc()
+        self._xi_break()
         self._episode_log = EpisodeLog(self.num_envs, b["ld"], capacity, self.torch_dtype, b["device"], self.env_id0)
         return self._episode_log
 
@@ -446,12 +503,15 @@
         RandomEnv.check_dr_violations(self)
 
     def get_task(self):
-        return self._alloc()["xi"][:self.num_envs]
+        b = self._alloc()
+        self._materialize_xi()
+        return b["xi"][:self.num_envs]
 
     def set_task(self, *task):
         b = self._alloc()
         t = _device.torch()
         n = self.num_envs
+        self._xi_break()
         if len(task) == 1:
             xi = t.as_tensor(task[0], device=b["device"]).to(self.torch_dtype)
             if xi.shape == (4,):
@@ -563,6 +623,7 @@
 
     def state_dict(self):
         b = self._alloc()
+        self._materialize_xi()
         out = {k: b[k].clone() for k in self._tensor_keys()}
         out.update(seed=self._seed, env_id0=self.env_id0, tick=self._tick, num_envs=self.num_envs,
                    dtype=self._dtype_name, lean=self.lean,
@@ -577,6 +638,7 @@
         if sd["num_envs"] != self.num_envs or sd["dtype"] != self._dtype_name or sd.get("lean", False) != self.lean:
             raise ValueError("state_dict is for %d %s envs%s" % (sd["num_envs"], sd["dtype"], " (lean)" if sd.get("lean") else ""))
         b = self._alloc()
+        self._xi_break()
         for k in self._tensor_keys():
             b[k].copy_(sd[k])
         self._seed, self.env_id0, self._tick = sd["seed"], sd["env_id0"], sd["tick"]
```

After: 97.16 billion (median of 6 runs). 5.2% higher.
